# Tencent/PocketFlow

Measured on AMD Instinct MI355X. Metric: images/sec ResNet-50 INT8 quant-aware fine-tune (whole job; per GPU = value / n_gpus), higher is better.
Workload: dtype bf16

## Files before the change

pocketflow_amd/csrc/pf_api.hip:

```cpp
#include "pf_common.h"

extern "C" int pf_version(void) { return 100; }

extern "C" const char* pf_error_string(int err) {
  if (err == 0) return "ok";
  return hipGetErrorString((hipError_t)err);
}

#include <stdlib.h>
#include <stdio.h>
static PfTuning g_tuning;
static bool g_tuning_loaded = false;

static int env_int(const char* name, int dflt) {
  const char* e = getenv(name);
  return (e == nullptr || *e == 0) ? dflt : atoi(e);
}

static void tuning_load() {
  PfTuning t;
  t.conv_bn = env_int("PF_CONV_BN", 0);
  t.conv_igemm = env_int("PF_CONV_IGEMM", 1);
  t.conv_igemm_pro = env_int("PF_CONV_IGEMM_PRO", 1);
  t.conv_stream = env_int("PF_CONV_STREAM", 1);
  t.conv_stream_maxsplit = env_int("PF_CONV_STREAM_MAXSPLIT", 2);
  t.igemm_pro3 = env_int("PF_IGEMM_PRO3", 1);
  t.igemm_tile_bm = t.igemm_tile_bn = 0;
  const char* e = getenv("PF_IGEMM_TILE");
  if (e != nullptr) {
    int bm = 0, bn = 0;
    if (sscanf(e, "%dx%d", &bm, &bn) == 2) { t.igemm_tile_bm = bm; t.igemm_tile_bn = bn; }
  }
  t.pool3s2 = env_int("PF_POOL3S2", 1);
  t.wrw_tr = env_int("PF_WRW_TR", 0);
  t.wrw2 = env_int("PF_WRW2", 1);
  t.wrw2_target = env_int("PF_WRW2_TARGET", 0);
  t.splitk = env_int("PF_IGEMM_SPLITK", 1);
  t.wrw2_tk256 = env_int("PF_WRW2_TK256", 1);
  t.conv3x3_c64 = env_int("PF_CONV3X3_C64", 1);
  g_tuning = t;
  g_tuning_loaded = true;
}

const PfTuning& pf_tuning() {
  if (!g_tuning_loaded) tuning_load();
  return g_tuning;
}

extern "C" int pf_tuning_reload(void) { tuning_load(); return 0; }

#include <map>
#include <mutex>
#include <utility>
int pf_require_lds(const void* fn, size_t lds) {
  static std::mutex mu;
  static std::map<std::pair<int, const void*>, size_t> done;
  int dev = 0;
  hipError_t e = hipGetDevice(&dev);
  if (e != hipSuccess) return (int)e;
  std::lock_guard<std::mutex> lock(mu);
  size_t& have = done[std::make_pair(dev, fn)];
  if (lds > have) {
    e = hipFuncSetAttribute(fn, hipFuncAttributeMaxDynamicSharedMemorySize, (int)lds);
    if (e != hipSuccess) return (int)e;
    have = lds;
  }
  return 0;
}
```

pocketflow_amd/csrc/pf_common.h:

```cpp
#pragma once
#include <hip/hip_runtime.h>
#include <stdint.h>
#include <type_traits>
#include "../../include/pocketflow_hip.h"

#define PF_WAVE 64
#define PF_THREADS 256
#define PF_MAX_GRID 2048

#define PF_LAUNCH_CHECK()                         \
  do {                                            \
    hipError_t e__ = hipGetLastError();           \
    if (e__ != hipSuccess) return (int)e__;       \
  } while (0)

typedef uint16_t bf16_t;

int pf_require_lds(const void* fn, size_t lds);

struct PfTuning {
  int conv_bn;
  int conv_igemm, conv_igemm_pro;
  int conv_stream;
  int conv_stream_maxsplit;
  int igemm_pro3;
  int igemm_tile_bm, igemm_tile_bn;
  int pool3s2;
  int wrw_tr, wrw2, wrw2_target;
  int wrw2_tk256;
  int splitk;
  int conv3x3_c64;
};
const PfTuning& pf_tuning();

__device__ __forceinline__ float bf16_to_f32(bf16_t h) {
  return __uint_as_float(((uint32_t)h) << 16);
}
__device__ __forceinline__ bf16_t f32_to_bf16(float f) {
  uint32_t u = __float_as_uint(f);
  if ((u & 0x7FFFFFFFu) > 0x7F800000u) return (bf16_t)((u >> 16) | 0x0040u);
  u += 0x7FFFu + ((u >> 16) & 1u);
  return (bf16_t)(u >> 16);
}

template <typename T> __device__ __forceinline__ float round_to(float v);
template <> __device__ __forceinline__ float round_to<float>(float v) { return v; }
template <> __device__ __forceinline__ float round_to<bf16_t>(float v) { return bf16_to_f32(f32_to_bf16(v)); }

template <typename T> struct VecTraits;
template <> struct VecTraits<float> { static constexpr int N = 4; };
template <> struct VecTraits<bf16_t> { static constexpr int N = 8; };

template <typename T>
__device__ __forceinline__ void load_vec(const T* __restrict__ p, float* out);
template <>
__device__ __forceinline__ void load_vec<float>(const float* __restrict__ p, float* out) {
  float4 v = *reinterpret_cast<const float4*>(p);
  out[0] = v.x; out[1] = v.y; out[2] = v.z; out[3] = v.w;
}
template <>
__device__ __forceinline__ void load_vec<bf16_t>(const bf16_t* __restrict__ p, float* out) {
  uint4 v = *reinterpret_cast<const uint4*>(p);
  out[0] = __uint_as_float(v.x << 16); out[1] = __uint_as_float(v.x & 0xFFFF0000u);
  out[2] = __uint_as_float(v.y << 16); out[3] = __uint_as_float(v.y & 0xFFFF0000u);
  out[4] = __uint_as_float(v.z << 16); out[5] = __uint_as_float(v.z & 0xFFFF0000u);
  out[6] = __uint_as_float(v.w << 16); out[7] = __uint_as_float(v.w & 0xFFFF0000u);
}
template <typename T>
__device__ __forceinline__ void store_vec(T* __restrict__ p, const float* in);
template <>
__device__ __forceinline__ void store_vec<float>(float* __restrict__ p, const float* in) {
  *reinterpret_cast<float4*>(p) = make_float4(in[0], in[1], in[2], in[3]);
}
template <>
__device__ __forceinline__ void store_vec<bf16_t>(bf16_t* __restrict__ p, const float* in) {
  uint4 v;
  v.x = (uint32_t)f32_to_bf16(in[0]) | ((uint32_t)f32_to_bf16(in[1]) << 16);
  v.y = (uint32_t)f32_to_bf16(in[2]) | ((uint32_t)f32_to_bf16(in[3]) << 16);
  v.z = (uint32_t)f32_to_bf16(in[4]) | ((uint32_t)f32_to_bf16(in[5]) << 16);
  v.w = (uint32_t)f32_to_bf16(in[6]) | ((uint32_t)f32_to_bf16(in[7]) << 16);
  *reinterpret_cast<uint4*>(p) = v;
}
template <typename T> __device__ __forceinline__ void load8(const T* __restrict__ p, float* out);
template <> __device__ __forceinline__ void load8<float>(const float* __restrict__ p, float* out) {
  load_vec<float>(p, out); load_vec<float>(p + 4, out + 4);
}
template <> __device__ __forceinline__ void load8<bf16_t>(const bf16_t* __restrict__ p, float* out) {
  load_vec<bf16_t>(p, out);
}
template <typename T> __device__ __forceinline__ void store8(T* __restrict__ p, const float* in);
template <> __device__ __forceinline__ void store8<float>(float* __restrict__ p, const float* in) {
  store_vec<float>(p, in); store_vec<float>(p + 4, in + 4);
}
template <> __device__ __forceinline__ void store8<bf16_t>(bf16_t* __restrict__ p, const float* in) {
  store_vec<bf16_t>(p, in);
}
__host__ __device__ __forceinline__ bool pf_aligned16(const void* p) {
  return (((uintptr_t)p) & 15) == 0;
}
template <typename T> __device__ __forceinline__ float load_one(const T* p);
template <> __device__ __forceinline__ float load_one<float>(const float* p) { return *p; }
template <> __device__ __forceinline__ float load_one<bf16_t>(const bf16_t* p) { return bf16_to_f32(*p); }
template <typename T> __device__ __forceinline__ void store_one(T* p, float v);
template <> __device__ __forceinline__ void store_one<float>(float* p, float v) { *p = v; }
template <> __device__ __forceinline__ void store_one<bf16_t>(bf16_t* p, float v) { *p = f32_to_bf16(v); }

__device__ __forceinline__ uint32_t enc_f32(float f) {
  uint32_t u = __float_as_uint(f);
  return (u & 0x80000000u) ? ~u : (u | 0x80000000u);
}
__device__ __forceinline__ float dec_f32(uint32_t e) {
  uint32_t u = (e & 0x80000000u) ? (e & 0x7FFFFFFFu) : ~e;
  return __uint_as_float(u);
}
__device__ __forceinline__ void slot_alpha_beta(const uint32_t* slot, float& alpha, float& beta) {
  const uint2 sv = *reinterpret_cast<const uint2*>(slot);
  float mn = dec_f32(sv.x);
  float mx = dec_f32(~sv.y);
  alpha = (mx - mn) + 1e-10f;
  beta = mn;
}

__device__ __forceinline__ float pf_acc_min(float a, float b) { float r; asm("v_min_f32 %0, %1, %2" : "=v"(r) : "v"(a), "v"(b)); return r; }
__device__ __forceinline__ float pf_acc_max(float a, float b) { float r; asm("v_max_f32 %0, %1, %2" : "=v"(r) : "v"(a), "v"(b)); return r; }

template <int ACT> __device__ __forceinline__ float apply_act(float x) {
  if (ACT == PF_ACT_RELU) return fmaxf(x, 0.0f);
  if (ACT == PF_ACT_RELU6) return fminf(fmaxf(x, 0.0f), 6.0f);
  return x;
}
template <int ACT> __device__ __forceinline__ float act_mask(float u) {
  if (ACT == PF_ACT_RELU) return u > 0.0f ? 1.0f : 0.0f;
  if (ACT == PF_ACT_RELU6) return (u > 0.0f && u < 6.0f) ? 1.0f : 0.0f;
  return 1.0f;
}

__device__ __forceinline__ float uq_point(float t, float alpha, float beta, float k) {
  float xn = (t - beta) / alpha;
  float q = rintf(xn * k) / k;
  return alpha * q + beta;
}
__host__ __device__ __forceinline__ float uq_k_of_bits(int bits) {
  return ldexpf(1.0f, bits) - 1.0f;
}

__device__ __forceinline__ float wave_min(float v) {
#pragma unroll
  for (int o = 32; o > 0; o >>= 1) v = fminf(v, __shfl_xor(v, o, 64));
  return v;
}
__device__ __forceinline__ float wave_max(float v) {
#pragma unroll
  for (int o = 32; o > 0; o >>= 1) v = fmaxf(v, __shfl_xor(v, o, 64));
  return v;
}
__device__ __forceinline__ float wave_sum(float v) {
#pragma unroll
  for (int o = 32; o > 0; o >>= 1) v += __shfl_xor(v, o, 64);
  return v;
}
__device__ __forceinline__ void block_minmax(float& mn, float& mx, float* lds ) {
  mn = wave_min(mn);
  mx = wave_max(mx);
  const int w = threadIdx.x >> 6, l = threadIdx.x & 63;
  if (l == 0) { lds[w] = mn; lds[4 + w] = mx; }
  __syncthreads();
  mn = fminf(fminf(lds[0], lds[1]), fminf(lds[2], lds[3]));
  mx = fmaxf(fmaxf(lds[4], lds[5]), fmaxf(lds[6], lds[7]));
  __syncthreads();
}
__device__ __forceinline__ float block_sum(float v, float* lds ) {
  v = wave_sum(v);
  const int w = threadIdx.x >> 6, l = threadIdx.x & 63;
  if (l == 0) lds[w] = v;
  __syncthreads();
  v = (lds[0] + lds[1]) + (lds[2] + lds[3]);
  __syncthreads();
  return v;
}

template <typename F> static inline void pf_with_act(int act, F&& f) {
  if (act == PF_ACT_RELU) f(std::integral_constant<int, PF_ACT_RELU>{});
  else if (act == PF_ACT_RELU6) f(std::integral_constant<int, PF_ACT_RELU6>{});
  else f(std::integral_constant<int, PF_ACT_NONE>{});
}
template <typename F> static inline void pf_with_bool(bool b, F&& f) {
  if (b) f(std::true_type{});
  else f(std::false_type{});
}

static inline int pf_grid_for(int64_t n, int per_block) {
  int64_t g = (n + per_block - 1) / per_block;
  if (g < 1) g = 1;
  if (g > PF_MAX_GRID) g = PF_MAX_GRID;
  return (int)g;
}
```

pocketflow_amd/csrc/pf_igemm.h:

```cpp
#pragma once
#include "pf_conv_common.h"

#define LDS_PTR(p) ((__attribute__((address_space(3))) void*)(p))

#if defined(__HIP_DEVICE_COMPILE__)
typedef __amdgpu_buffer_rsrc_t pf_rsrc_t;
#define PF_MAKE_RSRC(p, bytes) __builtin_amdgcn_make_buffer_rsrc((void*)(p), (short)0, (int)(bytes), 0x00020000)
#define PF_BUFFER_LOAD_LDS16(rs, lds, voff, soff) __builtin_amdgcn_raw_ptr_buffer_load_lds(rs, LDS_PTR(lds), 16, voff, soff, 0, 0)
#else
typedef int pf_rsrc_t;
#define PF_MAKE_RSRC(p, bytes) 0
#define PF_BUFFER_LOAD_LDS16(rs, lds, voff, soff) ((void)(rs), (void)(lds), (void)(voff), (void)(soff))
#endif

struct IgArgs {
  const bf16_t* X;
  const bf16_t* W;
  bf16_t* Y;
  const bf16_t* zero;
  uint32_t x_bytes, w_bytes;
  const bf16_t* R;
  float* partial;
  const bf16_t* bx;
  const float* bss;
  const float* bmi;
  float b_lo, b_hi;
  const float* ss;
  const uint32_t* slot;
  float kq, act_lo, act_hi;
  int M, N, C;
  int th, tw;
  int H, Wd, Ho, Wo, stride, pad_h, pad_w;
  int tiles_m, tiles_n, G;
  int w_r0, w_rs, w_s0, w_ss, w_S, w_taps_full;
  int o_sub, o_y, o_x, o_H, o_W;
  const float* oss;
  int oact;
  int rHo, rWo, rH, rW, rstride;
};

template <int N> __device__ __forceinline__ void wait_vm() { asm volatile("s_waitcnt vmcnt(%0)" ::"n"(N) : "memory"); }

#define IG_PLAIN 0
#define IG_BWD 1
#define IG_PRO 2
```

pocketflow_amd/csrc/pf_igemm.hip:

```cpp
#include "pf_conv_common.h"
#include <stdio.h>
#include <stdlib.h>

#include "pf_igemm.h"

#ifndef PF_IG_ABLATE
#define PF_IG_ABLATE 0
#endif
#define PF_IG_NO_DMA (PF_IG_ABLATE == 2 || PF_IG_ABLATE == 3 || PF_IG_ABLATE == 4)
#define PF_IG_FAKE_FRAGS (PF_IG_ABLATE == 3 || PF_IG_ABLATE == 4)

#ifdef PF_IG_TIMING
#define PF_IG_STAMP(k) do { if (tm_tile == 2) tmk[k] = (uint32_t)__builtin_readcyclecounter(); } while (0)
#else
#define PF_IG_STAMP(k) do { } while (0)
#endif

#ifdef PF_IG_CODES
#define PF_IG_XB 1
__device__ __forceinline__ bf16x8 ig_codes_to_bf16x8(uint2 c) {
  uint32_t r[4];
#pragma unroll
  for (int h = 0; h < 2; ++h) {
    const uint32_t w = h ? c.y : c.x;
    const float f0 = (float)(w & 0xffu), f1 = (float)((w >> 8) & 0xffu), f2 = (float)((w >> 16) & 0xffu), f3 = (float)(w >> 24);
    r[h * 2 + 0] = __builtin_amdgcn_perm(__float_as_uint(f1), __float_as_uint(f0), 0x07060302u);
    r[h * 2 + 1] = __builtin_amdgcn_perm(__float_as_uint(f3), __float_as_uint(f2), 0x07060302u);
  }
  const uint4 u = make_uint4(r[0], r[1], r[2], r[3]);
  return *reinterpret_cast<const bf16x8*>(&u);
}
#else
#define PF_IG_XB 2
#endif

template <int BM, int BN, int WM, int WN, int NS, int MODE, bool SUB = false, bool AFF = false, bool RMAP = false, bool BR = false>
__global__ __launch_bounds__(64 * WM * WN) void k_igemm(const IgArgs a) {
  constexpr bool BWD = (MODE == IG_BWD), PRO = (MODE == IG_PRO);
  static_assert(!BR || BWD, "BR is a variant of IG_BWD");
  static_assert(!PRO || NS == 2 || NS == 3, "the in-LDS prologue pass is written for the 2- and 3-stage rings");
  constexpr bool PRO3 = PRO && NS == 3;
  constexpr int NWC = WM * WN;
  constexpr int T = 64 * NWC;
  constexpr int TS = T;
  constexpr int TE = T;
  constexpr int WR = BM / WM, WC = BN / WN;
  constexpr int JM = WR / 16, NI = WC / 16;
  constexpr int XB = PF_IG_XB;
  constexpr int ACH = 4 * XB, AROW = 64 * XB;
  constexpr int AS = BM * ACH / TS, BS = BN * 8 / TS;
  constexpr int A_BYTES = BM * AROW, B_BYTES = BN * 128, STAGE = A_BYTES + B_BYTES;
  constexpr int CS_LD = BN + 8, CS_LD_B = BN + 8;
  constexpr int VPR = BN / 8, RPP = TE / VPR, NP = BM / RPP;
  static_assert(AS >= 1 && BS >= 1 && NP >= 1, "tile too small for the block");
  constexpr int LPS = AS + BS;
  extern __shared__ __attribute__((aligned(16))) unsigned char smem[];
  bf16_t* Cs = reinterpret_cast<bf16_t*>(smem);
  float* red = reinterpret_cast<float*>(smem);
  constexpr int RING_B = NS * STAGE, CT_B = BM * CS_LD_B * 2;
  float* bpl = reinterpret_cast<float*>(smem + (RING_B > CT_B ? RING_B : CT_B));
  float* ssl = bpl;

  const int tid = threadIdx.x, lane = tid & 63;
  const int wave = __builtin_amdgcn_readfirstlane(tid >> 6);
  const int swave = wave;
  const int cwave = wave % NWC;
  const int wm = cwave / WN, wn = cwave % WN;
  const int l15 = lane & 15, q = lane >> 4;
  const int srow = (swave * 64 + lane) >> 3;
  const int schunk = (lane & 7) ^ ((lane >> 3) & 7);
  const int srowA = (XB == 2) ? srow : ((swave * 64 + lane) >> 2);
  const int schunkA = (XB == 2) ? schunk : ((lane & 3) ^ ((lane >> 4) & 3));

  const int xcd = blockIdx.x & 7, L = blockIdx.x >> 3;
  const int g = xcd + 8 * (L / a.tiles_n), tn = L % a.tiles_n;
  const int n0 = tn * BN;
  const int cch = a.C >> 6;
  const int taps = a.th * a.tw;
  const int nk = taps * cch;
  const int64_t wrow = (int64_t)(SUB ? a.w_taps_full : taps) * a.C;
  const int hw_o = a.Ho * a.Wo;

  if (BWD) {
    for (int i = tid; i < 4 * BN; i += T) {
      const int qq = i / BN, c = n0 + (i - qq * BN);
      float v = 0.f;
      if (c < a.N) v = (qq < 2) ? a.bss[qq * a.N + c] : a.bmi[(qq - 2) * a.N + c];
      bpl[i] = v;
    }
  }

  float st_s[8], st_q[8], st_mn[8], st_mx[8];
#pragma unroll
  for (int j = 0; j < 8; ++j) { st_s[j] = 0.f; st_q[j] = 0.f; st_mn[j] = INFINITY; st_mx[j] = -INFINITY; }
  const int wvec = tid % VPR, wrw = tid / VPR;
  const bf16_t* __restrict__ side = BWD ? a.bx : nullptr;
  Pro pro;
  pro_init(pro, a.act_lo, a.act_hi, a.kq, PRO ? a.slot : nullptr);
  if (PRO3) {
    for (int i = tid; i < 2 * a.C; i += T) ssl[i] = (i < a.C) ? pro_fold_scale(pro, a.ss[i]) : pro_fold_shift(pro, a.ss[i]);
    __syncthreads();
  }

  const pf_rsrc_t rsX = PF_MAKE_RSRC(a.X, a.x_bytes);
  const pf_rsrc_t rsW = PF_MAKE_RSRC(a.W, a.w_bytes);
  constexpr uint32_t OOB = 0x80000000u;
  uint32_t boff[BS];
#pragma unroll
  for (int i = 0; i < BS; ++i) {
    const int n = n0 + i * (TS / 8) + srow;
    boff[i] = (n < a.N) ? (uint32_t)(((int64_t)n * wrow + schunk * 8) * 2) : OOB;
  }

  const bool pointwise = a.th == 1 && a.tw == 1 && a.stride == 1 && a.pad_h == 0 && a.pad_w == 0 && a.Ho == a.H && a.Wo == a.Wd;
  constexpr bool XPRE = !BWD && NS == 3 && 2 * STAGE >= BM * CS_LD_B * 2;
  constexpr int RB0 = XPRE ? 2 : 0;
  uint32_t pbase[AS], pmask[AS];
  int s_r = 0, s_s = 0, s_cc = 0, s_ks = 0, s_tap = 0;
  auto setup_tile = [&](int m0) {
#pragma unroll
    for (int i = 0; i < AS; ++i) {
      const int m = m0 + i * (TS / ACH) + srowA;
      pbase[i] = 0; pmask[i] = 0;
      if (pointwise) {
        if (m < a.M) { pbase[i] = (uint32_t)(m * a.C + schunkA * (16 / XB)) * (uint32_t)XB; pmask[i] = 1u; }
      } else if (m < a.M) {
        const int img = m / hw_o, rem = m - img * hw_o;
        const int ho = rem / a.Wo, wo = rem - ho * a.Wo;
        const int h0 = ho * a.stride - a.pad_h, w0 = wo * a.stride - a.pad_w;
        pbase[i] = (uint32_t)(((img * a.H + h0) * a.Wd + w0) * a.C + schunkA * (16 / XB)) * (uint32_t)XB;
        uint32_t mk = 0;
        for (int r = 0; r < a.th; ++r)
          for (int sx = 0; sx < a.tw; ++sx)
            if ((unsigned)(h0 + r) < (unsigned)a.H && (unsigned)(w0 + sx) < (unsigned)a.Wd) mk |= 1u << (r * a.tw + sx);
        pmask[i] = mk;
      }
    }
    s_r = 0; s_s = 0; s_cc = 0; s_ks = 0; s_tap = 0;
  };
  auto stage = [&](int buf) {
    unsigned char* As = smem + buf * STAGE;
    unsigned char* Bs = As + A_BYTES;
    const uint32_t tapoff = (uint32_t)(((s_r * a.Wd + s_s) * a.C + s_cc * 64) * XB);
#if !PF_IG_NO_DMA
#pragma unroll
    for (int i = 0; i < AS; ++i) {
      const uint32_t voff = ((pmask[i] >> s_tap) & 1u) ? (pbase[i] + tapoff) : OOB;
      PF_BUFFER_LOAD_LDS16(rsX, As + (i * (TS / ACH) + swave * (64 / ACH)) * AROW, voff, 0);
    }
    uint32_t woff = (uint32_t)(s_ks * 128);
    if constexpr (SUB) woff = (uint32_t)((((a.w_r0 + s_r * a.w_rs) * a.w_S + a.w_s0 + s_s * a.w_ss) * a.C + s_cc * 64) * 2);
#pragma unroll
    for (int i = 0; i < BS; ++i)
      PF_BUFFER_LOAD_LDS16(rsW, Bs + (i * (TS / 8) + swave * 8) * 128, boff[i], woff);
#else
    (void)As; (void)Bs; (void)tapoff;
#endif
    ++s_ks;
    if (++s_cc == cch) { s_cc = 0; ++s_tap; if (++s_s == a.tw) { s_s = 0; ++s_r; } }
  };
  bool pre = false;
#ifdef PF_IG_TIMING
  uint32_t tmk[16];
  int tm_tile = -1;
#pragma unroll
  for (int k = 0; k < 16; ++k) tmk[k] = 0;
#endif
  for (int tm = g; tm < a.tiles_m; tm += a.G) {
    const int m0 = tm * BM;
#ifdef PF_IG_TIMING
    ++tm_tile;
#endif
    PF_IG_STAMP(0);
    if (!pre) setup_tile(m0);

    f32x4 acc[NI][JM];
#pragma unroll
    for (int i = 0; i < NI; ++i)
#pragma unroll
      for (int j = 0; j < JM; ++j) acc[i][j] = (f32x4){0.f, 0.f, 0.f, 0.f};
    uint2 rr[NI][JM];
    const bool has_r = BWD ? BR : (a.R != nullptr);
    constexpr bool RPRE = BM * BN <= 128 * 256;
    auto load_residual = [&]() {
#pragma unroll
      for (int j = 0; j < JM; ++j) {
        const int m = m0 + wm * WR + j * 16 + l15;
        int64_t rrow = m;
        bool live = m < a.M;
        if constexpr (RMAP) {
          rrow = live ? rmap_row(m, a.rHo, a.rWo, a.rH, a.rW, a.rstride) : -1;
          live = rrow >= 0;
        }
#pragma unroll
        for (int i = 0; i < NI; ++i) {
          const int n = n0 + wn * WC + i * 16 + q * 4;
          rr[i][j] = make_uint2(0, 0);
          if (live && n < a.N) rr[i][j] = *reinterpret_cast<const uint2*>(a.R + rrow * a.N + n);
        }
      }
    };
    auto add_residual = [&](auto& c) {
#pragma unroll
      for (int j = 0; j < JM; ++j)
#pragma unroll
        for (int i = 0; i < NI; ++i) {
          c[i][j][0] += __uint_as_float(rr[i][j].x << 16); c[i][j][1] += __uint_as_float(rr[i][j].x & 0xFFFF0000u);
          c[i][j][2] += __uint_as_float(rr[i][j].y << 16); c[i][j][3] += __uint_as_float(rr[i][j].y & 0xFFFF0000u);
        }
    };

    int ibuf = RB0;
    float4 ps0 = make_float4(0, 0, 0, 0), ps1 = ps0, ph0 = ps0, ph1 = ps0;
    auto fetch_ss = [&](int cc) {
      const float* p = a.ss + cc * 64 + schunk * 8;
      ps0 = *reinterpret_cast<const float4*>(p); ps1 = *reinterpret_cast<const float4*>(p + 4);
      ph0 = *reinterpret_cast<const float4*>(p + a.C); ph1 = *reinterpret_cast<const float4*>(p + a.C + 4);
    };
    auto transform3 = [&](int buf, int cc, int i0, int i1) {
      const uint32_t pss = lds_addr(ssl + cc * 64 + schunk * 8);
      float4 s0, s1, h0, h1;
      if (i1 - i0 == 1 || i1 - i0 == 2) {
        const uint32_t pd = lds_addr(smem + buf * STAGE + srow * 128 + (lane & 7) * 16) + (uint32_t)(i0 * (TS / 8) * 128);
        uint4 v0, v1 = make_uint4(0, 0, 0, 0);
        if (i1 - i0 == 1) lds_read_b128x4_1(pss, pss + (uint32_t)a.C * 4u, pd, s0, s1, h0, h1, v0);
        else lds_read_b128x4_2(pss, pss + (uint32_t)a.C * 4u, pd, pd + (TS / 8) * 128, s0, s1, h0, h1, v0, v1);
        pro.sc[0] = s0.x; pro.sc[1] = s0.y; pro.sc[2] = s0.z; pro.sc[3] = s0.w;
        pro.sc[4] = s1.x; pro.sc[5] = s1.y; pro.sc[6] = s1.z; pro.sc[7] = s1.w;
        pro.sh[0] = h0.x; pro.sh[1] = h0.y; pro.sh[2] = h0.z; pro.sh[3] = h0.w;
        pro.sh[4] = h1.x; pro.sh[5] = h1.y; pro.sh[6] = h1.z; pro.sh[7] = h1.w;
        lds_write_b128(pd, pro_apply(pro, v0));
        if (i1 - i0 == 2) lds_write_b128(pd + (TS / 8) * 128, pro_apply(pro, v1));
        return;
      }
      lds_read_b128x4(pss, pss + (uint32_t)a.C * 4u, s0, s1, h0, h1);
      pro.sc[0] = s0.x; pro.sc[1] = s0.y; pro.sc[2] = s0.z; pro.sc[3] = s0.w;
      pro.sc[4] = s1.x; pro.sc[5] = s1.y; pro.sc[6] = s1.z; pro.sc[7] = s1.w;
      pro.sh[0] = h0.x; pro.sh[1] = h0.y; pro.sh[2] = h0.z; pro.sh[3] = h0.w;
      pro.sh[4] = h1.x; pro.sh[5] = h1.y; pro.sh[6] = h1.z; pro.sh[7] = h1.w;
      const uint32_t pv = lds_addr(smem + buf * STAGE + srow * 128 + (lane & 7) * 16);
      static_assert(!PRO3 || AS == 1 || AS == 2 || AS == 4 || AS == 8, "vector count per lane");
#pragma unroll
      for (int i = 0; i < AS; i += 2) {
        if (i >= i0 && i < i1) {
          if (i + 1 < i1) {
            uint4 v0, v1;
            lds_read_b128x2(pv + i * (TS / 8) * 128, pv + (i + 1) * (TS / 8) * 128, v0, v1);
            lds_write_b128(pv + i * (TS / 8) * 128, pro_apply(pro, v0));
            lds_write_b128(pv + (i + 1) * (TS / 8) * 128, pro_apply(pro, v1));
          } else {
            lds_write_b128(pv + i * (TS / 8) * 128, pro_apply(pro, lds_read_b128(pv + i * (TS / 8) * 128)));
          }
        } else if (i + 1 >= i0 && i + 1 < i1) {
          lds_write_b128(pv + (i + 1) * (TS / 8) * 128, pro_apply(pro, lds_read_b128(pv + (i + 1) * (TS / 8) * 128)));
        }
      }
    };
    auto transform = [&](int buf) {
      const float rs[8] = {ps0.x, ps0.y, ps0.z, ps0.w, ps1.x, ps1.y, ps1.z, ps1.w};
      const float rh[8] = {ph0.x, ph0.y, ph0.z, ph0.w, ph1.x, ph1.y, ph1.z, ph1.w};
#pragma unroll
      for (int j = 0; j < 8; ++j) { pro.sc[j] = pro_fold_scale(pro, rs[j]); pro.sh[j] = pro_fold_shift(pro, rh[j]); }
      unsigned char* As = smem + buf * STAGE;
#pragma unroll
      for (int i = 0; i < AS; ++i) {
        uint4* p = reinterpret_cast<uint4*>(As + (i * (TS / 8) + srow) * 128 + (lane & 7) * 16);
        *p = pro_apply(pro, *p);
      }
    };
    {
#pragma unroll
    for (int d = 0; d < NS - 1; ++d)
      if (d < nk) {
        if (d > 0 || !pre) {
          if (PRO && !PRO3) fetch_ss(s_cc);
          stage(ibuf);
        }
        ibuf = (ibuf + 1 == NS) ? 0 : ibuf + 1;
      }
    PF_IG_STAMP(1);
    if (nk >= NS - 1) wait_vm<(NS - 2) * LPS>(); else wait_vm<0>();
    PF_IG_STAMP(2);
    if (PRO3) { transform3(RB0, 0, 0, AS); asm volatile("s_waitcnt lgkmcnt(0)" ::: "memory"); }
    else if (PRO) { transform(RB0); asm volatile("s_waitcnt lgkmcnt(0)" ::: "memory"); }
    __builtin_amdgcn_s_barrier();
    PF_IG_STAMP(3);
    int cbuf = RB0;
    for (int ks = 0; ks < nk; ++ks) {
      const bool more = ks + NS - 1 < nk;
      const int tbuf = ibuf;
      if (more) {
        if (PRO && !PRO3) fetch_ss(s_cc);
        stage(ibuf);
        ibuf = (ibuf + 1 == NS) ? 0 : ibuf + 1;
      }
      const unsigned char* As = smem + cbuf * STAGE;
      const unsigned char* Bs = As + A_BYTES;
      cbuf = (cbuf + 1 == NS) ? 0 : cbuf + 1;
      const bool tnext = PRO3 && (ks + 1 < nk);
      if (PRO3) {
        if (more) wait_vm<LPS>(); else if (ks + 1 < nk) wait_vm<0>();
      }
      if (RPRE && has_r && ks == ((PRO3 && nk >= 2) ? nk - 2 : nk - 1)) load_residual();
#pragma unroll
      for (int kk = 0; kk < 2; ++kk) {
        const int coff = (((kk * 4 + q) ^ (l15 & 7)) << 4);
        bf16x8 wf[NI], xf[JM];
#if PF_IG_ABLATE != 1
#if PF_IG_FAKE_FRAGS
#pragma unroll
        for (int i = 0; i < NI; ++i) { uint4 u = make_uint4(lane, i, kk, 0x3f803f80u); asm volatile("" : "+v"(u.x)); wf[i] = *reinterpret_cast<const bf16x8*>(&u); }
#pragma unroll
        for (int j = 0; j < JM; ++j) { uint4 u = make_uint4(lane, j, kk, 0x3f803f80u); asm volatile("" : "+v"(u.x)); xf[j] = *reinterpret_cast<const bf16x8*>(&u); }
        (void)coff;
#else
#pragma unroll
        for (int i = 0; i < NI; ++i)
          wf[i] = *reinterpret_cast<const bf16x8*>(Bs + (wn * WC + i * 16 + l15) * 128 + coff);
#ifdef PF_IG_CODES
        const int coffA = ((((kk * 2 + (q >> 1)) ^ ((l15 >> 2) & 3)) << 4) + (q & 1) * 8);
#pragma unroll
        for (int j = 0; j < JM; ++j)
          xf[j] = ig_codes_to_bf16x8(*reinterpret_cast<const uint2*>(As + (wm * WR + j * 16 + l15) * AROW + coffA));
#else
#pragma unroll
        for (int j = 0; j < JM; ++j)
          xf[j] = *reinterpret_cast<const bf16x8*>(As + (wm * WR + j * 16 + l15) * 128 + coff);
#endif
#endif
#pragma unroll
        for (int i = 0; i < NI; ++i)
#pragma unroll
          for (int j = 0; j < JM; ++j)
            acc[i][j] = __builtin_amdgcn_mfma_f32_16x16x32_bf16(wf[i], xf[j], acc[i][j], 0, 0, 0);
        if constexpr (NI == 4 && JM == 4 && PRO3) {
          __builtin_amdgcn_sched_group_barrier(0x100, NI + JM, 0);
          __builtin_amdgcn_sched_group_barrier(0x008, NI * JM, 0);
        }
        if constexpr ((NI == 4 || NI == 2) && JM == 4 && !PRO3) {
          if (kk == 1) {
            __builtin_amdgcn_sched_group_barrier(0x100, NI + JM, 0);
#pragma unroll
            for (int i = 0; i < NI + JM; ++i) {
              __builtin_amdgcn_sched_group_barrier(0x008, (NI * JM) / (NI + JM), 0);
              __builtin_amdgcn_sched_group_barrier(0x100, 1, 0);
            }
            __builtin_amdgcn_sched_group_barrier(0x008, NI * JM - (NI + JM) * ((NI * JM) / (NI + JM)) + NI * JM, 0);
          }
        }
#else
        (void)coff; (void)wf; (void)xf;
#endif
        if (tnext) transform3(cbuf, ks + 1, kk * (AS / 2), (kk == 1) ? AS : (AS / 2));
      }
      if (!PRO3) {
        if (more) wait_vm<(NS - 2) * LPS>(); else wait_vm<0>();
      }
      if (PRO && !PRO3 && more) transform(tbuf);
      asm volatile("s_waitcnt lgkmcnt(0)" ::: "memory");
      __builtin_amdgcn_s_barrier();
      __builtin_amdgcn_sched_barrier(0);
#ifdef PF_IG_TIMING
      if (ks < 4) PF_IG_STAMP(4 + ks);
      if (ks == nk - 1) PF_IG_STAMP(8);
#endif
    }
    }

#if PF_IG_ABLATE >= 4
    {
      if (a.M < 0) {
#pragma unroll
        for (int i = 0; i < NI; ++i)
#pragma unroll
          for (int j = 0; j < JM; ++j) reinterpret_cast<uint32_t*>(a.Y)[(i * JM + j) * 64 + lane] = pack_bf16x2(acc[i][j][0] + acc[i][j][1], acc[i][j][2] + acc[i][j][3]);
      }
      continue;
    }
#endif
    {
    if (has_r) {
      if constexpr (RPRE) add_residual(acc);
      else {
#pragma unroll
        for (int j = 0; j < JM; ++j) {
          const int m = m0 + wm * WR + j * 16 + l15;
          int64_t rrow = m;
          bool live = m < a.M;
          if constexpr (RMAP) {
            rrow = live ? rmap_row(m, a.rHo, a.rWo, a.rH, a.rW, a.rstride) : -1;
            live = rrow >= 0;
          }
#pragma unroll
          for (int i = 0; i < NI; ++i) {
            const int n = n0 + wn * WC + i * 16 + q * 4;
            if (live && n < a.N) {
              const uint2 r = *reinterpret_cast<const uint2*>(a.R + rrow * a.N + n);
              acc[i][j][0] += __uint_as_float(r.x << 16); acc[i][j][1] += __uint_as_float(r.x & 0xFFFF0000u);
              acc[i][j][2] += __uint_as_float(r.y << 16); acc[i][j][3] += __uint_as_float(r.y & 0xFFFF0000u);
            }
          }
          __builtin_amdgcn_sched_barrier(0);
        }
      }
    }
    PF_IG_STAMP(9);
    pre = false;
    if constexpr (XPRE) {
      __builtin_amdgcn_sched_barrier(0);
      if (tm + a.G < a.tiles_m) {
        setup_tile((tm + a.G) * BM);
        stage(RB0);
        pre = true;
      }
      __builtin_amdgcn_sched_barrier(0);
    }
#ifdef PF_IG_CODES
#pragma unroll
    for (int i = 0; i < NI; ++i)
#pragma unroll
      for (int j = 0; j < JM; ++j)
#pragma unroll
        for (int e = 0; e < 4; ++e) acc[i][j][e] *= a.kq;
#endif
#pragma unroll
    for (int i = 0; i < NI; ++i)
#pragma unroll
      for (int j = 0; j < JM; ++j) {
        const uint2 v = make_uint2(pack_bf16x2(acc[i][j][0], acc[i][j][1]), pack_bf16x2(acc[i][j][2], acc[i][j][3]));
        if constexpr (XPRE) lds_write_b64(lds_addr(Cs + (wm * WR + j * 16 + l15) * CS_LD + wn * WC + i * 16 + q * 4), v);
        else *reinterpret_cast<uint2*>(Cs + (wm * WR + j * 16 + l15) * CS_LD + wn * WC + i * 16 + q * 4) = v;
      }
    }
    constexpr int PG = (NP > 8) ? 8 : NP;
    uint4 rres[PG];
    auto load_side = [&](int p0) {
#pragma unroll
      for (int p = 0; p < PG; ++p) {
        const int m = m0 + wrw + (p0 + p) * RPP, n = n0 + wvec * 8;
        rres[p] = make_uint4(0, 0, 0, 0);
        if (m < a.M && n < a.N) {
          int64_t srow = m;
          if constexpr (SUB) {
            const int oimg = m / hw_o, orem = m - oimg * hw_o;
            const int oi = orem / a.Wo, oj = orem - oi * a.Wo;
            srow = ((int64_t)oimg * a.o_H + oi * a.o_sub + a.o_y) * a.o_W + oj * a.o_sub + a.o_x;
          }
          rres[p] = *reinterpret_cast<const uint4*>(side + srow * a.N + n);
        }
      }
    };
    constexpr bool etid = true;
    float bpr[32];
    if (BWD && !BR) {
#pragma unroll
      for (int qq = 0; qq < 4; ++qq)
#pragma unroll
        for (int j = 0; j < 8; ++j) bpr[qq * 8 + j] = bpl[qq * BN + wvec * 8 + j];
    }
    if (side != nullptr && etid) load_side(0);
    PF_IG_STAMP(10);
    if constexpr (XPRE) { asm volatile("s_waitcnt lgkmcnt(0)" ::: "memory"); __builtin_amdgcn_s_barrier(); __builtin_amdgcn_sched_barrier(0); }
    else __syncthreads();
    PF_IG_STAMP(11);
#pragma unroll
    for (int p0 = 0; p0 < NP; p0 += PG) {
      u32x4_t cv[8];
      if constexpr (XPRE && PG == 8) {
#pragma unroll
        for (int pp = 0; pp < PG; ++pp) lds_read_b128_nowait(lds_addr(Cs + (wrw + (p0 + pp) * RPP) * CS_LD + wvec * 8), cv[pp]);
        lds_wait_batch8(cv);
      } else {
#pragma unroll
        for (int pp = 0; pp < PG; ++pp) cv[pp] = *reinterpret_cast<const u32x4_t*>(Cs + (wrw + (p0 + pp) * RPP) * CS_LD + wvec * 8);
      }
#pragma unroll
      for (int pp = 0; pp < PG; ++pp) {
        const int p = p0 + pp;
        const int rl = wrw + p * RPP;
        const int m = m0 + rl, n = n0 + wvec * 8;
        if (m < a.M && n < a.N && etid) {
          uint4 c;
          c = make_uint4(cv[pp][0], cv[pp][1], cv[pp][2], cv[pp][3]);
          if (BWD) {
            float f[8], xv[8];
            unpack8(c, f);
            unpack8(rres[pp], xv);
            const float* bp = BR ? (bpl + wvec * 8) : bpr;
            constexpr int BPS = BR ? BN : 8;
#pragma unroll
            for (int j = 0; j < 8; ++j) {
              const float u = fmaf(bp[j], xv[j], bp[BPS + j]);
              const float dy = (u > a.b_lo && u < a.b_hi) ? f[j] : 0.f;
              st_s[j] += dy;
              st_q[j] = fmaf(dy, (xv[j] - bp[2 * BPS + j]) * bp[3 * BPS + j], st_q[j]);
            }
          } else if (a.R != nullptr || a.partial != nullptr) {
            float f[8];
            unpack8(c, f);
            if (a.partial != nullptr) {
#pragma unroll
              for (int j = 0; j < 8; ++j) {
                st_s[j] += f[j];
                st_q[j] = fmaf(f[j], f[j], st_q[j]);
                st_mn[j] = pf_acc_min(st_mn[j], f[j]);
                st_mx[j] = pf_acc_max(st_mx[j], f[j]);
              }
            }
          }
          if constexpr (AFF) c = out_affine8(c, a.oss, a.N, n, a.oact);
          int64_t orow = m;
          if constexpr (SUB) {
            const int oimg = m / hw_o, orem = m - oimg * hw_o;
            const int oi = orem / a.Wo, oj = orem - oi * a.Wo;
            orow = ((int64_t)oimg * a.o_H + oi * a.o_sub + a.o_y) * a.o_W + oj * a.o_sub + a.o_x;
          }
          *reinterpret_cast<uint4*>(a.Y + orow * a.N + n) = c;
        }
      }
      if (side != nullptr && p0 + PG < NP && etid) load_side(p0 + PG);
    }
    PF_IG_STAMP(12);
    if constexpr (XPRE) { asm volatile("s_waitcnt lgkmcnt(0)" ::: "memory"); __builtin_amdgcn_s_barrier(); __builtin_amdgcn_sched_barrier(0); }
    else __syncthreads();
    PF_IG_STAMP(13);
#ifdef PF_IG_TIMING
    if (tm_tile == 2 && blockIdx.x == gridDim.x / 2 && tid == 0) {
      uint32_t* out = reinterpret_cast<uint32_t*>(const_cast<bf16_t*>(a.zero));
#pragma unroll
      for (int k = 0; k < 14; ++k) out[k] = tmk[k];
      out[14] = (uint32_t)__builtin_readcyclecounter();
    }
#endif
  }

  if (a.partial != nullptr) {
    constexpr int nstat_max = 4;
    const int nstat = BWD ? 2 : 4;
    __syncthreads();
    for (int stat = 0; stat < nstat; ++stat) {
      const float* v = (stat == 0) ? st_s : (stat == 1 ? st_q : (stat == 2 ? st_mn : st_mx));
#pragma unroll
      for (int j = 0; j < 8; ++j) red[wrw * BN + wvec * 8 + j] = v[j];
      __syncthreads();
      for (int c = tid; c < BN; c += T) {
        float r = red[c];
        for (int rr = 1; rr < RPP; ++rr) {
          const float w = red[rr * BN + c];
          r = (stat < 2) ? (r + w) : (stat == 2 ? fminf(r, w) : fmaxf(r, w));
        }
        if (n0 + c < a.N) a.partial[((int64_t)g * nstat + stat) * a.N + n0 + c] = r;
      }
      __syncthreads();
    }
    (void)nstat_max;
  }
}

static IgCfg ig_pick(int M, int N, bool pro) {
  if (pro) {
    if (pf_tuning().igemm_pro3 != 0) {
      if (N % 256 == 0) return IgCfg{128, 256, 256, true};
      if (N % 128 == 0) return IgCfg{256, 128, 256, true};
    }
    return IgCfg{128, (N % 128 == 0) ? 128 : 64, 512, false};
  }
  {
    const int bm = pf_tuning().igemm_tile_bm, bn = pf_tuning().igemm_tile_bn;
    if ((bm == 128 || bm == 256) && (bn == 64 || bn == 128) && (N % bn == 0 || bn == 64))
      return IgCfg{bm, bn, (bm == 256) ? 256 : 512, false};
  }
  const int bn = (N % 128 == 0) ? 128 : 64;
  return IgCfg{128, bn, 512, false};
}

static IgArgs ig_args_plain(int th, int tw) {
  IgArgs a;
  a.X = nullptr; a.W = nullptr; a.Y = nullptr; a.zero = nullptr; a.x_bytes = 0; a.w_bytes = 0;
  a.R = nullptr; a.partial = nullptr; a.bx = nullptr; a.bss = nullptr; a.bmi = nullptr; a.b_lo = -INFINITY; a.b_hi = INFINITY;
  a.ss = nullptr; a.slot = nullptr; a.kq = 255.f; a.act_lo = -INFINITY; a.act_hi = INFINITY;
  a.M = 0; a.N = 0; a.C = 0; a.th = th; a.tw = tw;
  a.H = 1; a.Wd = 1; a.Ho = 1; a.Wo = 1; a.stride = 1; a.pad_h = 0; a.pad_w = 0;
  a.tiles_m = 0; a.tiles_n = 0; a.G = 0;
  a.w_r0 = 0; a.w_rs = 1; a.w_s0 = 0; a.w_ss = 1; a.w_S = tw; a.w_taps_full = th * tw;
  a.o_sub = 0; a.o_y = 0; a.o_x = 0; a.o_H = 0; a.o_W = 0;
  a.oss = nullptr; a.oact = PF_ACT_NONE;
  a.rHo = 0; a.rWo = 0; a.rH = 0; a.rW = 0; a.rstride = 1;
  return a;
}

template <int BM, int BN, int WM, int WN, int NS, int MODE, bool SUB = false, bool AFF = false, bool RMAP = false, bool BR = false>
static int ig_launch_t(IgArgs& a, int slots, hipStream_t st) {
  constexpr bool BWD = (MODE == IG_BWD), PRO3 = (MODE == IG_PRO && NS == 3);
  constexpr int THREADS = 64 * WM * WN;
  a.tiles_m = (a.M + BM - 1) / BM;
  a.tiles_n = (a.N + BN - 1) / BN;
  const int planned_G = a.G;
  const int grid = pf_conv_grid(slots, a.tiles_m, a.tiles_n, &a.G);
  if (planned_G > 0 && a.G != planned_G) return (int)hipErrorInvalidValue;
  constexpr size_t ring = NS * (size_t)(BM + BN) * 128, ctile = (size_t)BM * (BN + 8) * 2;
  constexpr size_t base = (ring > ctile ? ring : ctile);
  const size_t lds = base + (BWD ? 4 * BN * 4 : 0) + (PRO3 ? 2 * (size_t)a.C * 4 : 0);
  if (PRO3 && a.C > CV_MAXK) return (int)hipErrorInvalidValue;
  const size_t lds_max = base + (BWD ? 4 * BN * 4 : 0) + (PRO3 ? 2 * (size_t)CV_MAXK * 4 : 0);
  if (int e = pf_require_lds(reinterpret_cast<const void*>(&k_igemm<BM, BN, WM, WN, NS, MODE, SUB, AFF, RMAP, BR>), lds_max)) return e;
  k_igemm<BM, BN, WM, WN, NS, MODE, SUB, AFF, RMAP, BR><<<grid, THREADS, lds, st>>>(a);
  PF_LAUNCH_CHECK();
  return 0;
}

bool pf_conv3x3_c64_geom(int H, int Wd, int C, int N, int th, int tw, int stride, int pad_h, int pad_w, int Ho, int Wo);
bool pf_conv3x3_c64_takes(const IgArgs& a);
int pf_conv3x3_c64_stats_groups(int M);
int pf_conv3x3_c64_launch(const IgArgs& a, hipStream_t st);

static bool ig_carries_affine(const IgCfg& c, bool pro, int taps) { return pro ? (c.pro3 && taps == 1) : c.bm == 128; }

static int ig_launch(IgArgs& a, const IgCfg& c, hipStream_t st) {
  const bool bwd = a.bx != nullptr, pro = a.ss != nullptr;
  if (pf_conv3x3_c64_takes(a)) return pf_conv3x3_c64_launch(a, st);
  if (a.oss != nullptr) {
    if (bwd) return (int)hipErrorInvalidValue;
    if (!ig_carries_affine(c, pro, a.th * a.tw)) {
      const float* oss = a.oss;
      a.oss = nullptr;
      const int r = ig_launch(a, c, st);
      if (r != 0) return r;
      return pf_bn_act_quant_apply(a.Y, a.Y, PF_BF16, a.M, a.N, oss, a.oact, nullptr, 8, 0, st);
    }
    if (pro) return (c.bn == 256) ? ig_launch_t<128, 256, 2, 4, 3, IG_PRO, false, true>(a, c.slots, st)
                                  : ig_launch_t<256, 128, 4, 2, 3, IG_PRO, false, true>(a, c.slots, st);
    return (c.bn == 128) ? ig_launch_t<128, 128, 2, 2, 2, IG_PLAIN, false, true>(a, c.slots, st)
                         : ig_launch_t<128, 64, 2, 2, 2, IG_PLAIN, false, true>(a, c.slots, st);
  }
  if (pro) {
    if (a.th * a.tw != 1 || bwd) return (int)hipErrorInvalidValue;
    if (c.pro3) return (c.bn == 256) ? ig_launch_t<128, 256, 2, 4, 3, IG_PRO>(a, c.slots, st)
                                     : ig_launch_t<256, 128, 4, 2, 3, IG_PRO>(a, c.slots, st);
    return (c.bn == 128) ? ig_launch_t<128, 128, 2, 2, 2, IG_PRO>(a, c.slots, st) : ig_launch_t<128, 64, 2, 2, 2, IG_PRO>(a, c.slots, st);
  }
#define PF_IG(BMV, BNV, WMV, WNV, NSV) (bwd ? ig_launch_t<BMV, BNV, WMV, WNV, NSV, IG_BWD>(a, c.slots, st) : ig_launch_t<BMV, BNV, WMV, WNV, NSV, IG_PLAIN>(a, c.slots, st))
  if (c.bm == 256 && c.bn == 128) return PF_IG(256, 128, 4, 2, 3);
  if (c.bm == 128 && c.bn == 128) return PF_IG(128, 128, 2, 2, 2);
  if (c.bm == 256 && c.bn == 64) return PF_IG(256, 64, 4, 1, 2);
  return PF_IG(128, 64, 2, 2, 2);
#undef PF_IG
}

extern "C" int pf_conv2d_stats_groups_geom(int imgs, int H, int Wd, int C, int N, int th, int tw, int stride, int pad_h,
                                           int pad_w, int Ho, int Wo) {
  if (pf_conv3x3_c64_geom(H, Wd, C, N, th, tw, stride, pad_h, pad_w, Ho, Wo) && (imgs * Ho * Wo) % (Ho * Wo) == 0)
    return pf_conv3x3_c64_stats_groups(imgs * Ho * Wo);
  const int M = imgs * Ho * Wo;
  const IgCfg c = ig_pick(M, N, false);
  int G;
  pf_conv_grid(c.slots, (M + c.bm - 1) / c.bm, (N + c.bn - 1) / c.bn, &G);
  return G;
}

static int conv2d_fwd_launch(const void* X, const void* W, void* Y, const void* zero, const void* R, float* partial,
                             const void* bn_x, const float* bn_scale_shift, const float* bn_mean_invstd, int bn_act,
                             int imgs, int H, int Wd, int C, int N, int th, int tw, int stride, int pad_h, int pad_w,
                             int Ho, int Wo, void* stream, const float* out_scale_shift, int out_act) {
  if (out_scale_shift != nullptr && (R != nullptr || partial != nullptr || bn_x != nullptr)) return (int)hipErrorInvalidValue;
  if (imgs <= 0 || H <= 0 || Wd <= 0 || Ho <= 0 || Wo <= 0 || C <= 0 || N <= 0 || (C % 64) || (N % 8) || th < 1 || tw < 1 ||
      stride < 1)
    return (int)hipErrorInvalidValue;
  if (!pf_aligned16(X) || !pf_aligned16(W) || !pf_aligned16(Y) || !pf_aligned16(zero) || zero == nullptr ||
      (R && !pf_aligned16(R)) || (bn_x && !pf_aligned16(bn_x)))
    return (int)hipErrorInvalidValue;
  if (bn_x != nullptr && (R != nullptr || partial == nullptr || bn_scale_shift == nullptr || bn_mean_invstd == nullptr))
    return (int)hipErrorInvalidValue;
  if ((int64_t)imgs * H * Wd * C >= ((int64_t)1 << 30) || (int64_t)N * th * tw * C >= ((int64_t)1 << 30) || th * tw > 32)
    return (int)hipErrorInvalidValue;
  IgArgs a = ig_args_plain(th, tw);
  a.X = (const bf16_t*)X; a.W = (const bf16_t*)W; a.Y = (bf16_t*)Y; a.zero = (const bf16_t*)zero;
  a.R = (const bf16_t*)R; a.partial = partial; a.bx = (const bf16_t*)bn_x; a.bss = bn_scale_shift; a.bmi = bn_mean_invstd;
  pf_act_window(bn_act, &a.b_lo, &a.b_hi);
  a.M = imgs * Ho * Wo; a.N = N; a.C = C;
  a.H = H; a.Wd = Wd; a.Ho = Ho; a.Wo = Wo; a.stride = stride; a.pad_h = pad_h; a.pad_w = pad_w;
  a.x_bytes = (uint32_t)((int64_t)imgs * H * Wd * C * 2);
  a.w_bytes = (uint32_t)((int64_t)N * th * tw * C * 2);
  a.oss = out_scale_shift; a.oact = out_act;
  return ig_launch(a, ig_pick(a.M, N, false), (hipStream_t)stream);
}

extern "C" int pf_conv2d_fwd(const void* X, const void* W, void* Y, const void* zero, const void* R, float* partial,
                             const void* bn_x, const float* bn_scale_shift, const float* bn_mean_invstd, int bn_act,
                             int imgs, int H, int Wd, int C, int N, int th, int tw, int stride, int pad_h, int pad_w,
                             int Ho, int Wo, void* stream) {
  return conv2d_fwd_launch(X, W, Y, zero, R, partial, bn_x, bn_scale_shift, bn_mean_invstd, bn_act, imgs, H, Wd, C, N, th, tw,
                           stride, pad_h, pad_w, Ho, Wo, stream, nullptr, PF_ACT_NONE);
}

#ifdef PF_IG_CODES
extern "C" int pf_probe_conv2d_fwd_codes(const void* Xc, float alpha, const void* W, void* Y, const void* zero, int imgs, int H,
                                         int Wd, int C, int N, int th, int tw, int stride, int pad_h, int pad_w, int Ho, int Wo,
                                         void* stream) {
  if ((C % 64) || (N % 64) || !pf_aligned16(Xc) || !pf_aligned16(W) || !pf_aligned16(Y)) return (int)hipErrorInvalidValue;
  IgArgs a = ig_args_plain(th, tw);
  a.X = (const bf16_t*)Xc; a.W = (const bf16_t*)W; a.Y = (bf16_t*)Y; a.zero = (const bf16_t*)zero;
  a.kq = alpha;
  a.M = imgs * Ho * Wo; a.N = N; a.C = C;
  a.H = H; a.Wd = Wd; a.Ho = Ho; a.Wo = Wo; a.stride = stride; a.pad_h = pad_h; a.pad_w = pad_w;
  a.x_bytes = (uint32_t)((int64_t)imgs * H * Wd * C);
  a.w_bytes = (uint32_t)((int64_t)N * th * tw * C * 2);
  const IgCfg c = ig_pick(a.M, a.N, false);
  if (c.bm == 256 && c.bn == 128) return ig_launch_t<256, 128, 4, 2, 3, IG_PLAIN>(a, c.slots, (hipStream_t)stream);
  if (c.bm == 128 && c.bn == 128) return ig_launch_t<128, 128, 2, 2, 2, IG_PLAIN>(a, c.slots, (hipStream_t)stream);
  if (c.bm == 256 && c.bn == 64) return ig_launch_t<256, 64, 4, 1, 2, IG_PLAIN>(a, c.slots, (hipStream_t)stream);
  return ig_launch_t<128, 64, 2, 2, 2, IG_PLAIN>(a, c.slots, (hipStream_t)stream);
}
#endif

extern "C" int pf_conv2d_fwd_affine(const void* X, const void* W, void* Y, const void* zero, const float* out_scale_shift,
                                    int out_act, int imgs, int H, int Wd, int C, int N, int th, int tw, int stride, int pad_h,
                                    int pad_w, int Ho, int Wo, void* stream) {
  if (out_scale_shift == nullptr) return (int)hipErrorInvalidValue;
  return conv2d_fwd_launch(X, W, Y, zero, nullptr, nullptr, nullptr, nullptr, nullptr, PF_ACT_NONE, imgs, H, Wd, C, N, th, tw,
                           stride, pad_h, pad_w, Ho, Wo, stream, out_scale_shift, out_act);
}

static int strided_class_groups(int imgs, int H, int Wd, int C, int stride) {
  const int bn = (C % 128 == 0) ? 128 : 64;
  int G;
  pf_conv_grid(512, (imgs * (H / stride) * (Wd / stride) + 127) / 128, (C + bn - 1) / bn, &G);
  return G;
}

extern "C" int pf_conv2d_bwd_data_strided_stats_groups(int imgs, int H, int Wd, int C, int stride) {
  if (imgs <= 0 || H <= 0 || Wd <= 0 || C <= 0 || stride < 2 || (H % stride) || (Wd % stride)) return 0;
  return stride * stride * strided_class_groups(imgs, H, Wd, C, stride);
}

static int strided_launch(const void* dY, const void* Wt, void* dX, const void* zero, int imgs, int H, int Wd, int C, int N, int R,
                          int S, int stride, int pad_h, int pad_w, int Ho, int Wo, void* stream, float* partial, const void* bn_x,
                          const float* bss, const float* bmi, int bn_act) {
  if (imgs <= 0 || H <= 0 || Wd <= 0 || Ho <= 0 || Wo <= 0 || C <= 0 || N <= 0 || (N % 64) || (C % 8) || stride < 2 || R < stride ||
      S < stride || (H % stride) || (Wd % stride) || pad_h < 0 || pad_w < 0 || R * S > 32)
    return (int)hipErrorInvalidValue;
  if (!pf_aligned16(dY) || !pf_aligned16(Wt) || !pf_aligned16(dX) || zero == nullptr) return (int)hipErrorInvalidValue;
  if ((int64_t)imgs * Ho * Wo * N >= ((int64_t)1 << 30) || (int64_t)C * R * S * N >= ((int64_t)1 << 30)) return (int)hipErrorInvalidValue;
  const int Hc = H / stride, Wc = Wd / stride;
  for (int ay = 0; ay < stride; ++ay) {
    for (int ax = 0; ax < stride; ++ax) {
      const int r1 = (ay + pad_h) % stride, s1 = (ax + pad_w) % stride;
      const int th = (R - r1 + stride - 1) / stride, tw = (S - s1 + stride - 1) / stride;
      const int dmin_h = (ay + pad_h - r1) / stride - (th - 1), dmin_w = (ax + pad_w - s1) / stride - (tw - 1);
      IgArgs a = ig_args_plain(th, tw);
      a.X = (const bf16_t*)dY; a.W = (const bf16_t*)Wt; a.Y = (bf16_t*)dX; a.zero = (const bf16_t*)zero;
      if (bn_x != nullptr) {
        a.partial = partial + (int64_t)(ay * stride + ax) * strided_class_groups(imgs, H, Wd, C, stride) * 2 * C;
        a.bx = (const bf16_t*)bn_x; a.bss = bss; a.bmi = bmi;
        pf_act_window(bn_act, &a.b_lo, &a.b_hi);
      }
      a.M = imgs * Hc * Wc; a.N = C; a.C = N;
      a.H = Ho; a.Wd = Wo; a.Ho = Hc; a.Wo = Wc; a.stride = 1; a.pad_h = -dmin_h; a.pad_w = -dmin_w;
      a.x_bytes = (uint32_t)((int64_t)imgs * Ho * Wo * N * 2);
      a.w_bytes = (uint32_t)((int64_t)C * R * S * N * 2);
      a.w_r0 = (R - 1 - r1) - (th - 1) * stride; a.w_rs = stride;
      a.w_s0 = (S - 1 - s1) - (tw - 1) * stride; a.w_ss = stride;
      a.w_S = S; a.w_taps_full = R * S;
      a.o_sub = stride; a.o_y = ay; a.o_x = ax; a.o_H = H; a.o_W = Wd;
      int rc;
      if (bn_x != nullptr)
        rc = (C % 128 == 0) ? ig_launch_t<128, 128, 2, 2, 2, IG_BWD, true>(a, 512, (hipStream_t)stream)
                            : ig_launch_t<128, 64, 2, 2, 2, IG_BWD, true>(a, 512, (hipStream_t)stream);
      else
        rc = (C % 128 == 0) ? ig_launch_t<128, 128, 2, 2, 2, IG_PLAIN, true>(a, 512, (hipStream_t)stream)
                            : ig_launch_t<128, 64, 2, 2, 2, IG_PLAIN, true>(a, 512, (hipStream_t)stream);
      if (rc != 0) return rc;
    }
  }
  return 0;
}

extern "C" int pf_conv2d_bwd_data_strided(const void* dY, const void* Wt, void* dX, const void* zero, int imgs, int H, int Wd,
                                          int C, int N, int R, int S, int stride, int pad_h, int pad_w, int Ho, int Wo, void* stream) {
  return strided_launch(dY, Wt, dX, zero, imgs, H, Wd, C, N, R, S, stride, pad_h, pad_w, Ho, Wo, stream, nullptr, nullptr, nullptr,
                        nullptr, PF_ACT_NONE);
}

extern "C" int pf_conv2d_bwd_data_strided_bnstats(const void* dY, const void* Wt, void* dX, const void* zero, const void* bn_x,
                                                  const float* bn_scale_shift, const float* bn_mean_invstd, int bn_act,
                                                  float* partial, int imgs, int H, int Wd, int C, int N, int R, int S, int stride,
                                                  int pad_h, int pad_w, int Ho, int Wo, void* stream) {
  if (bn_x == nullptr || partial == nullptr || bn_scale_shift == nullptr || bn_mean_invstd == nullptr || !pf_aligned16(bn_x))
    return (int)hipErrorInvalidValue;
  return strided_launch(dY, Wt, dX, zero, imgs, H, Wd, C, N, R, S, stride, pad_h, pad_w, Ho, Wo, stream, partial, bn_x,
                        bn_scale_shift, bn_mean_invstd, bn_act);
}

bool pf_igemm_conv1x1_plan(const Conv1x1Req& q, Conv1x1Plan* p) {
  const int64_t lim = (int64_t)1 << 30;
  if ((q.K % 64) || q.rows_in * q.K >= lim || (int64_t)q.N * q.K >= lim) return false;
  IgCfg c = ig_pick(q.M, q.N, q.pro);
  if (q.join) {
    if ((q.N % 64) || c.bm != 128 || c.slots != 512 || c.bn != ((q.N % 128 == 0) ? 128 : 64)) return false;
    if (q.ymap || q.map || !q.res || q.pro || q.aff) return false;
  } else if (q.ymap) {
    if ((q.N % 64) || q.rows_out * q.N >= lim) return false;
    c = IgCfg{128, (q.N % 128 == 0) ? 128 : 64, 512, false};
  }
  p->kernel = CONV_IGEMM;
  p->ig = c;
  p->grid = pf_conv_grid(c.slots, (q.M + c.bm - 1) / c.bm, (q.N + c.bn - 1) / c.bn, &p->G);
  p->rows_in = q.rows_in;
  p->affine_after = q.aff && !ig_carries_affine(c, q.pro, 1);
  return true;
}

int pf_igemm_conv1x1(const ConvArgs& c, const Conv1x1Plan& p, hipStream_t st) {
  const bool rowmap = c.stride > 1 && !c.ymap;
  IgArgs a = ig_args_plain(1, 1);
  a.X = c.X; a.W = c.W; a.Y = c.Y; a.zero = c.X;
#ifdef PF_IG_TIMING
  a.zero = (const bf16_t*)(uintptr_t)strtoull(getenv("PF_IG_TIMING_PTR"), nullptr, 0);
#endif
  a.R = c.R; a.partial = c.partial; a.bx = c.bx; a.bss = c.bss; a.bmi = c.bmi; a.b_lo = c.b_lo; a.b_hi = c.b_hi;
  a.ss = c.ss; a.slot = c.slot; a.kq = c.kq; a.act_lo = c.act_lo; a.act_hi = c.act_hi;
  a.M = c.M; a.N = c.N; a.C = c.K; a.G = p.G;
  if (c.ymap) { a.H = c.Ho; a.Wd = c.Wo; a.Ho = c.Ho; a.Wo = c.Wo; }
  else if (rowmap) { a.H = c.H; a.Wd = c.Wd; a.Ho = c.Ho; a.Wo = c.Wo; a.stride = c.stride; }
  a.x_bytes = (uint32_t)(p.rows_in * c.K * 2);
  a.w_bytes = (uint32_t)((int64_t)c.N * c.K * 2);
  a.oss = c.oss; a.oact = c.oact;
  a.rHo = c.rHo; a.rWo = c.rWo; a.rH = c.rH; a.rW = c.rW; a.rstride = c.rstride;
  const bool rmap = a.rstride > 1, br = a.bx != nullptr && a.R != nullptr, wide = (p.ig.bn == 128);
  if (rmap || br) {
    if (!br) return wide ? ig_launch_t<128, 128, 2, 2, 2, IG_PLAIN, false, false, true, false>(a, 512, st)
                         : ig_launch_t<128, 64, 2, 2, 2, IG_PLAIN, false, false, true, false>(a, 512, st);
    if (rmap) return wide ? ig_launch_t<128, 128, 2, 2, 2, IG_BWD, false, false, true, true>(a, 512, st)
                          : ig_launch_t<128, 64, 2, 2, 2, IG_BWD, false, false, true, true>(a, 512, st);
    return wide ? ig_launch_t<128, 128, 2, 2, 2, IG_BWD, false, false, false, true>(a, 512, st)
                : ig_launch_t<128, 64, 2, 2, 2, IG_BWD, false, false, false, true>(a, 512, st);
  }
  if (c.ymap) {
    a.o_sub = c.stride; a.o_y = 0; a.o_x = 0; a.o_H = c.H; a.o_W = c.Wd;
    return wide ? ig_launch_t<128, 128, 2, 2, 2, IG_PLAIN, true>(a, 512, st) : ig_launch_t<128, 64, 2, 2, 2, IG_PLAIN, true>(a, 512, st);
  }
  return ig_launch(a, p.ig, st);
}
```

Before: 11620.

## Fuse strided backward-data sub-convolution classes into a single kernel launch

Adds an IgSubArgs struct carrying up to 16 per-phase sub-class descriptors (tap offsets, padding, output offsets, partial pointers). The igemm kernel now loops over these classes internally, so a strided transposed convolution needs one launch instead of one per phase. This targets the per-launch overhead and the tail effects of many small grids. In exchange the kernel grows larger, and per-block work becomes uneven when classes have different tap counts.

```diff
diff --git a/pocketflow_amd/csrc/pf_api.hip b/pocketflow_amd/csrc/pf_api.hip
--- a/pocketflow_amd/csrc/pf_api.hip
+++ b/pocketflow_amd/csrc/pf_api.hip
@@ -38,6 +38,7 @@
   t.splitk = env_int("PF_IGEMM_SPLITK", 1);
   t.wrw2_tk256 = env_int("PF_WRW2_TK256", 1);
   t.conv3x3_c64 = env_int("PF_CONV3X3_C64", 1);
+  t.strided_one_launch = env_int("PF_STRIDED_ONE_LAUNCH", 1);
   g_tuning = t;
   g_tuning_loaded = true;
 }
diff --git a/pocketflow_amd/csrc/pf_common.h b/pocketflow_amd/csrc/pf_common.h
--- a/pocketflow_amd/csrc/pf_common.h
+++ b/pocketflow_amd/csrc/pf_common.h
@@ -30,6 +30,7 @@
   int wrw2_tk256;
   int splitk;
   int conv3x3_c64;
+  int strided_one_launch;
 };
 const PfTuning& pf_tuning();
 
diff --git a/pocketflow_amd/csrc/pf_igemm.h b/pocketflow_amd/csrc/pf_igemm.h
--- a/pocketflow_amd/csrc/pf_igemm.h
+++ b/pocketflow_amd/csrc/pf_igemm.h
@@ -12,6 +12,16 @@
 #define PF_MAKE_RSRC(p, bytes) 0
 #define PF_BUFFER_LOAD_LDS16(rs, lds, voff, soff) ((void)(rs), (void)(lds), (void)(voff), (void)(soff))
 #endif
+
+#define IG_MAX_CLS 16
+struct IgSubCls {
+  int th, tw, pad_h, pad_w;
+  int w_r0, w_s0;
+  int o_y, o_x;
+  int rot;
+  int pad_;
+  float* partial;
+};
 
 struct IgArgs {
   const bf16_t* X;
@@ -39,6 +49,12 @@
   int rHo, rWo, rH, rW, rstride;
 };
 
+struct IgSubArgs : IgArgs {
+  int n_cls;
+  IgSubCls cls[IG_MAX_CLS];
+};
+template <bool SUB, class A> __device__ __forceinline__ const A& ig_sub_args(const A& a) { return a; }
+
 template <int N> __device__ __forceinline__ void wait_vm() { asm volatile("s_waitcnt vmcnt(%0)" ::"n"(N) : "memory"); }
 
 #define IG_PLAIN 0
diff --git a/pocketflow_amd/csrc/pf_igemm.hip b/pocketflow_amd/csrc/pf_igemm.hip
--- a/pocketflow_amd/csrc/pf_igemm.hip
+++ b/pocketflow_amd/csrc/pf_igemm.hip
@@ -36,525 +36,14 @@
 
 template <int BM, int BN, int WM, int WN, int NS, int MODE, bool SUB = false, bool AFF = false, bool RMAP = false, bool BR = false>
 __global__ __launch_bounds__(64 * WM * WN) void k_igemm(const IgArgs a) {
-  constexpr bool BWD = (MODE == IG_BWD), PRO = (MODE == IG_PRO);
-  static_assert(!BR || BWD, "BR is a variant of IG_BWD");
-  static_assert(!PRO || NS == 2 || NS == 3, "the in-LDS prologue pass is written for the 2- and 3-stage rings");
-  constexpr bool PRO3 = PRO && NS == 3;
-  constexpr int NWC = WM * WN;
-  constexpr int T = 64 * NWC;
-  constexpr int TS = T;
-  constexpr int TE = T;
-  constexpr int WR = BM / WM, WC = BN / WN;
-  constexpr int JM = WR / 16, NI = WC / 16;
-  constexpr int XB = PF_IG_XB;
-  constexpr int ACH = 4 * XB, AROW = 64 * XB;
-  constexpr int AS = BM * ACH / TS, BS = BN * 8 / TS;
-  constexpr int A_BYTES = BM * AROW, B_BYTES = BN * 128, STAGE = A_BYTES + B_BYTES;
-  constexpr int CS_LD = BN + 8, CS_LD_B = BN + 8;
-  constexpr int VPR = BN / 8, RPP = TE / VPR, NP = BM / RPP;
-  static_assert(AS >= 1 && BS >= 1 && NP >= 1, "tile too small for the block");
-  constexpr int LPS = AS + BS;
-  extern __shared__ __attribute__((aligned(16))) unsigned char smem[];
-  bf16_t* Cs = reinterpret_cast<bf16_t*>(smem);
-  float* red = reinterpret_cast<float*>(smem);
-  constexpr int RING_B = NS * STAGE, CT_B = BM * CS_LD_B * 2;
-  float* bpl = reinterpret_cast<float*>(smem + (RING_B > CT_B ? RING_B : CT_B));
-  float* ssl = bpl;
-
-  const int tid = threadIdx.x, lane = tid & 63;
-  const int wave = __builtin_amdgcn_readfirstlane(tid >> 6);
-  const int swave = wave;
-  const int cwave = wave % NWC;
-  const int wm = cwave / WN, wn = cwave % WN;
-  const int l15 = lane & 15, q = lane >> 4;
-  const int srow = (swave * 64 + lane) >> 3;
-  const int schunk = (lane & 7) ^ ((lane >> 3) & 7);
-  const int srowA = (XB == 2) ? srow : ((swave * 64 + lane) >> 2);
-  const int schunkA = (XB == 2) ? schunk : ((lane & 3) ^ ((lane >> 4) & 3));
-
-  const int xcd = blockIdx.x & 7, L = blockIdx.x >> 3;
-  const int g = xcd + 8 * (L / a.tiles_n), tn = L % a.tiles_n;
-  const int n0 = tn * BN;
-  const int cch = a.C >> 6;
-  const int taps = a.th * a.tw;
-  const int nk = taps * cch;
-  const int64_t wrow = (int64_t)(SUB ? a.w_taps_full : taps) * a.C;
-  const int hw_o = a.Ho * a.Wo;
-
-  if (BWD) {
-    for (int i = tid; i < 4 * BN; i += T) {
-      const int qq = i / BN, c = n0 + (i - qq * BN);
-      float v = 0.f;
-      if (c < a.N) v = (qq < 2) ? a.bss[qq * a.N + c] : a.bmi[(qq - 2) * a.N + c];
-      bpl[i] = v;
-    }
-  }
-
-  float st_s[8], st_q[8], st_mn[8], st_mx[8];
-#pragma unroll
-  for (int j = 0; j < 8; ++j) { st_s[j] = 0.f; st_q[j] = 0.f; st_mn[j] = INFINITY; st_mx[j] = -INFINITY; }
-  const int wvec = tid % VPR, wrw = tid / VPR;
-  const bf16_t* __restrict__ side = BWD ? a.bx : nullptr;
-  Pro pro;
-  pro_init(pro, a.act_lo, a.act_hi, a.kq, PRO ? a.slot : nullptr);
-  if (PRO3) {
-    for (int i = tid; i < 2 * a.C; i += T) ssl[i] = (i < a.C) ? pro_fold_scale(pro, a.ss[i]) : pro_fold_shift(pro, a.ss[i]);
-    __syncthreads();
-  }
-
-  const pf_rsrc_t rsX = PF_MAKE_RSRC(a.X, a.x_bytes);
-  const pf_rsrc_t rsW = PF_MAKE_RSRC(a.W, a.w_bytes);
-  constexpr uint32_t OOB = 0x80000000u;
-  uint32_t boff[BS];
-#pragma unroll
-  for (int i = 0; i < BS; ++i) {
-    const int n = n0 + i * (TS / 8) + srow;
-    boff[i] = (n < a.N) ? (uint32_t)(((int64_t)n * wrow + schunk * 8) * 2) : OOB;
-  }
-
-  const bool pointwise = a.th == 1 && a.tw == 1 && a.stride == 1 && a.pad_h == 0 && a.pad_w == 0 && a.Ho == a.H && a.Wo == a.Wd;
-  constexpr bool XPRE = !BWD && NS == 3 && 2 * STAGE >= BM * CS_LD_B * 2;
-  constexpr int RB0 = XPRE ? 2 : 0;
-  uint32_t pbase[AS], pmask[AS];
-  int s_r = 0, s_s = 0, s_cc = 0, s_ks = 0, s_tap = 0;
-  auto setup_tile = [&](int m0) {
-#pragma unroll
-    for (int i = 0; i < AS; ++i) {
-      const int m = m0 + i * (TS / ACH) + srowA;
-      pbase[i] = 0; pmask[i] = 0;
-      if (pointwise) {
-        if (m < a.M) { pbase[i] = (uint32_t)(m * a.C + schunkA * (16 / XB)) * (uint32_t)XB; pmask[i] = 1u; }
-      } else if (m < a.M) {
-        const int img = m / hw_o, rem = m - img * hw_o;
-        const int ho = rem / a.Wo, wo = rem - ho * a.Wo;
-        const int h0 = ho * a.stride - a.pad_h, w0 = wo * a.stride - a.pad_w;
-        pbase[i] = (uint32_t)(((img * a.H + h0) * a.Wd + w0) * a.C + schunkA * (16 / XB)) * (uint32_t)XB;
-        uint32_t mk = 0;
-        for (int r = 0; r < a.th; ++r)
-          for (int sx = 0; sx < a.tw; ++sx)
-            if ((unsigned)(h0 + r) < (unsigned)a.H && (unsigned)(w0 + sx) < (unsigned)a.Wd) mk |= 1u << (r * a.tw + sx);
-        pmask[i] = mk;
-      }
-    }
-    s_r = 0; s_s = 0; s_cc = 0; s_ks = 0; s_tap = 0;
-  };
-  auto stage = [&](int buf) {
-    unsigned char* As = smem + buf * STAGE;
-    unsigned char* Bs = As + A_BYTES;
-    const uint32_t tapoff = (uint32_t)(((s_r * a.Wd + s_s) * a.C + s_cc * 64) * XB);
-#if !PF_IG_NO_DMA
-#pragma unroll
-    for (int i = 0; i < AS; ++i) {
-      const uint32_t voff = ((pmask[i] >> s_tap) & 1u) ? (pbase[i] + tapoff) : OOB;
-      PF_BUFFER_LOAD_LDS16(rsX, As + (i * (TS / ACH) + swave * (64 / ACH)) * AROW, voff, 0);
-    }
-    uint32_t woff = (uint32_t)(s_ks * 128);
-    if constexpr (SUB) woff = (uint32_t)((((a.w_r0 + s_r * a.w_rs) * a.w_S + a.w_s0 + s_s * a.w_ss) * a.C + s_cc * 64) * 2);
-#pragma unroll
-    for (int i = 0; i < BS; ++i)
-      PF_BUFFER_LOAD_LDS16(rsW, Bs + (i * (TS / 8) + swave * 8) * 128, boff[i], woff);
-#else
-    (void)As; (void)Bs; (void)tapoff;
-#endif
-    ++s_ks;
-    if (++s_cc == cch) { s_cc = 0; ++s_tap; if (++s_s == a.tw) { s_s = 0; ++s_r; } }
-  };
-  bool pre = false;
-#ifdef PF_IG_TIMING
-  uint32_t tmk[16];
-  int tm_tile = -1;
-#pragma unroll
-  for (int k = 0; k < 16; ++k) tmk[k] = 0;
-#endif
-  for (int tm = g; tm < a.tiles_m; tm += a.G) {
-    const int m0 = tm * BM;
-#ifdef PF_IG_TIMING
-    ++tm_tile;
-#endif
-    PF_IG_STAMP(0);
-    if (!pre) setup_tile(m0);
-
-    f32x4 acc[NI][JM];
-#pragma unroll
-    for (int i = 0; i < NI; ++i)
-#pragma unroll
-      for (int j = 0; j < JM; ++j) acc[i][j] = (f32x4){0.f, 0.f, 0.f, 0.f};
-    uint2 rr[NI][JM];
-    const bool has_r = BWD ? BR : (a.R != nullptr);
-    constexpr bool RPRE = BM * BN <= 128 * 256;
-    auto load_residual = [&]() {
-#pragma unroll
-      for (int j = 0; j < JM; ++j) {
-        const int m = m0 + wm * WR + j * 16 + l15;
-        int64_t rrow = m;
-        bool live = m < a.M;
-        if constexpr (RMAP) {
-          rrow = live ? rmap_row(m, a.rHo, a.rWo, a.rH, a.rW, a.rstride) : -1;
-          live = rrow >= 0;
-        }
-#pragma unroll
-        for (int i = 0; i < NI; ++i) {
-          const int n = n0 + wn * WC + i * 16 + q * 4;
-          rr[i][j] = make_uint2(0, 0);
-          if (live && n < a.N) rr[i][j] = *reinterpret_cast<const uint2*>(a.R + rrow * a.N + n);
-        }
-      }
-    };
-    auto add_residual = [&](auto& c) {
-#pragma unroll
-      for (int j = 0; j < JM; ++j)
-#pragma unroll
-        for (int i = 0; i < NI; ++i) {
-          c[i][j][0] += __uint_as_float(rr[i][j].x << 16); c[i][j][1] += __uint_as_float(rr[i][j].x & 0xFFFF0000u);
-          c[i][j][2] += __uint_as_float(rr[i][j].y << 16); c[i][j][3] += __uint_as_float(rr[i][j].y & 0xFFFF0000u);
-        }
-    };
-
-    int ibuf = RB0;
-    float4 ps0 = make_float4(0, 0, 0, 0), ps1 = ps0, ph0 = ps0, ph1 = ps0;
-    auto fetch_ss = [&](int cc) {
-      const float* p = a.ss + cc * 64 + schunk * 8;
-      ps0 = *reinterpret_cast<const float4*>(p); ps1 = *reinterpret_cast<const float4*>(p + 4);
-      ph0 = *reinterpret_cast<const float4*>(p + a.C); ph1 = *reinterpret_cast<const float4*>(p + a.C + 4);
-    };
-    auto transform3 = [&](int buf, int cc, int i0, int i1) {
-      const uint32_t pss = lds_addr(ssl + cc * 64 + schunk * 8);
-      float4 s0, s1, h0, h1;
-      if (i1 - i0 == 1 || i1 - i0 == 2) {
-        const uint32_t pd = lds_addr(smem + buf * STAGE + srow * 128 + (lane & 7) * 16) + (uint32_t)(i0 * (TS / 8) * 128);
-        uint4 v0, v1 = make_uint4(0, 0, 0, 0);
-        if (i1 - i0 == 1) lds_read_b128x4_1(pss, pss + (uint32_t)a.C * 4u, pd, s0, s1, h0, h1, v0);
-        else lds_read_b128x4_2(pss, pss + (uint32_t)a.C * 4u, pd, pd + (TS / 8) * 128, s0, s1, h0, h1, v0, v1);
-        pro.sc[0] = s0.x; pro.sc[1] = s0.y; pro.sc[2] = s0.z; pro.sc[3] = s0.w;
-        pro.sc[4] = s1.x; pro.sc[5] = s1.y; pro.sc[6] = s1.z; pro.sc[7] = s1.w;
-        pro.sh[0] = h0.x; pro.sh[1] = h0.y; pro.sh[2] = h0.z; pro.sh[3] = h0.w;
-        pro.sh[4] = h1.x; pro.sh[5] = h1.y; pro.sh[6] = h1.z; pro.sh[7] = h1.w;
-        lds_write_b128(pd, pro_apply(pro, v0));
-        if (i1 - i0 == 2) lds_write_b128(pd + (TS / 8) * 128, pro_apply(pro, v1));
-        return;
-      }
-      lds_read_b128x4(pss, pss + (uint32_t)a.C * 4u, s0, s1, h0, h1);
-      pro.sc[0] = s0.x; pro.sc[1] = s0.y; pro.sc[2] = s0.z; pro.sc[3] = s0.w;
-      pro.sc[4] = s1.x; pro.sc[5] = s1.y; pro.sc[6] = s1.z; pro.sc[7] = s1.w;
-      pro.sh[0] = h0.x; pro.sh[1] = h0.y; pro.sh[2] = h0.z; pro.sh[3] = h0.w;
-      pro.sh[4] = h1.x; pro.sh[5] = h1.y; pro.sh[6] = h1.z; pro.sh[7] = h1.w;
-      const uint32_t pv = lds_addr(smem + buf * STAGE + srow * 128 + (lane & 7) * 16);
-      static_assert(!PRO3 || AS == 1 || AS == 2 || AS == 4 || AS == 8, "vector count per lane");
-#pragma unroll
-      for (int i = 0; i < AS; i += 2) {
-        if (i >= i0 && i < i1) {
-          if (i + 1 < i1) {
-            uint4 v0, v1;
-            lds_read_b128x2(pv + i * (TS / 8) * 128, pv + (i + 1) * (TS / 8) * 128, v0, v1);
-            lds_write_b128(pv + i * (TS / 8) * 128, pro_apply(pro, v0));
-            lds_write_b128(pv + (i + 1) * (TS / 8) * 128, pro_apply(pro, v1));
-          } else {
-            lds_write_b128(pv + i * (TS / 8) * 128, pro_apply(pro, lds_read_b128(pv + i * (TS / 8) * 128)));
-          }
-        } else if (i + 1 >= i0 && i + 1 < i1) {
-          lds_write_b128(pv + (i + 1) * (TS / 8) * 128, pro_apply(pro, lds_read_b128(pv + (i + 1) * (TS / 8) * 128)));
-        }
-      }
-    };
-    auto transform = [&](int buf) {
-      const float rs[8] = {ps0.x, ps0.y, ps0.z, ps0.w, ps1.x, ps1.y, ps1.z, ps1.w};
-      const float rh[8] = {ph0.x, ph0.y, ph0.z, ph0.w, ph1.x, ph1.y, ph1.z, ph1.w};
-#pragma unroll
-      for (int j = 0; j < 8; ++j) { pro.sc[j] = pro_fold_scale(pro, rs[j]); pro.sh[j] = pro_fold_shift(pro, rh[j]); }
-      unsigned char* As = smem + buf * STAGE;
-#pragma unroll
-      for (int i = 0; i < AS; ++i) {
-        uint4* p = reinterpret_cast<uint4*>(As + (i * (TS / 8) + srow) * 128 + (lane & 7) * 16);
-        *p = pro_apply(pro, *p);
-      }
-    };
-    {
-#pragma unroll
-    for (int d = 0; d < NS - 1; ++d)
-      if (d < nk) {
-        if (d > 0 || !pre) {
-          if (PRO && !PRO3) fetch_ss(s_cc);
-          stage(ibuf);
-        }
-        ibuf = (ibuf + 1 == NS) ? 0 : ibuf + 1;
-      }
-    PF_IG_STAMP(1);
-    if (nk >= NS - 1) wait_vm<(NS - 2) * LPS>(); else wait_vm<0>();
-    PF_IG_STAMP(2);
-    if (PRO3) { transform3(RB0, 0, 0, AS); asm volatile("s_waitcnt lgkmcnt(0)" ::: "memory"); }
-    else if (PRO) { transform(RB0); asm volatile("s_waitcnt lgkmcnt(0)" ::: "memory"); }
-    __builtin_amdgcn_s_barrier();
-    PF_IG_STAMP(3);
-    int cbuf = RB0;
-    for (int ks = 0; ks < nk; ++ks) {
-      const bool more = ks + NS - 1 < nk;
-      const int tbuf = ibuf;
-      if (more) {
-        if (PRO && !PRO3) fetch_ss(s_cc);
-        stage(ibuf);
-        ibuf = (ibuf + 1 == NS) ? 0 : ibuf + 1;
-      }
-      const unsigned char* As = smem + cbuf * STAGE;
-      const unsigned char* Bs = As + A_BYTES;
-      cbuf = (cbuf + 1 == NS) ? 0 : cbuf + 1;
-      const bool tnext = PRO3 && (ks + 1 < nk);
-      if (PRO3) {
-        if (more) wait_vm<LPS>(); else if (ks + 1 < nk) wait_vm<0>();
-      }
-      if (RPRE && has_r && ks == ((PRO3 && nk >= 2) ? nk - 2 : nk - 1)) load_residual();
-#pragma unroll
-      for (int kk = 0; kk < 2; ++kk) {
-        const int coff = (((kk * 4 + q) ^ (l15 & 7)) << 4);
-        bf16x8 wf[NI], xf[JM];
-#if PF_IG_ABLATE != 1
-#if PF_IG_FAKE_FRAGS
-#pragma unroll
-        for (int i = 0; i < NI; ++i) { uint4 u = make_uint4(lane, i, kk, 0x3f803f80u); asm volatile("" : "+v"(u.x)); wf[i] = *reinterpret_cast<const bf16x8*>(&u); }
-#pragma unroll
-        for (int j = 0; j < JM; ++j) { uint4 u = make_uint4(lane, j, kk, 0x3f803f80u); asm volatile("" : "+v"(u.x)); xf[j] = *reinterpret_cast<const bf16x8*>(&u); }
-        (void)coff;
-#else
-#pragma unroll
-        for (int i = 0; i < NI; ++i)
-          wf[i] = *reinterpret_cast<const bf16x8*>(Bs + (wn * WC + i * 16 + l15) * 128 + coff);
-#ifdef PF_IG_CODES
-        const int coffA = ((((kk * 2 + (q >> 1)) ^ ((l15 >> 2) & 3)) << 4) + (q & 1) * 8);
-#pragma unroll
-        for (int j = 0; j < JM; ++j)
-          xf[j] = ig_codes_to_bf16x8(*reinterpret_cast<const uint2*>(As + (wm * WR + j * 16 + l15) * AROW + coffA));
-#else
-#pragma unroll
-        for (int j = 0; j < JM; ++j)
-          xf[j] = *reinterpret_cast<const bf16x8*>(As + (wm * WR + j * 16 + l15) * 128 + coff);
-#endif
-#endif
-#pragma unroll
-        for (int i = 0; i < NI; ++i)
-#pragma unroll
-          for (int j = 0; j < JM; ++j)
-            acc[i][j] = __builtin_amdgcn_mfma_f32_16x16x32_bf16(wf[i], xf[j], acc[i][j], 0, 0, 0);
-        if constexpr (NI == 4 && JM == 4 && PRO3) {
-          __builtin_amdgcn_sched_group_barrier(0x100, NI + JM, 0);
-          __builtin_amdgcn_sched_group_barrier(0x008, NI * JM, 0);
-        }
-        if constexpr ((NI == 4 || NI == 2) && JM == 4 && !PRO3) {
-          if (kk == 1) {
-            __builtin_amdgcn_sched_group_barrier(0x100, NI + JM, 0);
-#pragma unroll
-            for (int i = 0; i < NI + JM; ++i) {
-              __builtin_amdgcn_sched_group_barrier(0x008, (NI * JM) / (NI + JM), 0);
-              __builtin_amdgcn_sched_group_barrier(0x100, 1, 0);
-            }
-            __builtin_amdgcn_sched_group_barrier(0x008, NI * JM - (NI + JM) * ((NI * JM) / (NI + JM)) + NI * JM, 0);
-          }
-        }
-#else
-        (void)coff; (void)wf; (void)xf;
-#endif
-        if (tnext) transform3(cbuf, ks + 1, kk * (AS / 2), (kk == 1) ? AS : (AS / 2));
-      }
-      if (!PRO3) {
-        if (more) wait_vm<(NS - 2) * LPS>(); else wait_vm<0>();
-      }
-      if (PRO && !PRO3 && more) transform(tbuf);
-      asm volatile("s_waitcnt lgkmcnt(0)" ::: "memory");
-      __builtin_amdgcn_s_barrier();
-      __builtin_amdgcn_sched_barrier(0);
-#ifdef PF_IG_TIMING
-      if (ks < 4) PF_IG_STAMP(4 + ks);
-      if (ks == nk - 1) PF_IG_STAMP(8);
-#endif
-    }
-    }
-
-#if PF_IG_ABLATE >= 4
-    {
-      if (a.M < 0) {
-#pragma unroll
-        for (int i = 0; i < NI; ++i)
-#pragma unroll
-          for (int j = 0; j < JM; ++j) reinterpret_cast<uint32_t*>(a.Y)[(i * JM + j) * 64 + lane] = pack_bf16x2(acc[i][j][0] + acc[i][j][1], acc[i][j][2] + acc[i][j][3]);
-      }
-      continue;
-    }
-#endif
-    {
-    if (has_r) {
-      if constexpr (RPRE) add_residual(acc);
-      else {
-#pragma unroll
-        for (int j = 0; j < JM; ++j) {
-          const int m = m0 + wm * WR + j * 16 + l15;
-          int64_t rrow = m;
-          bool live = m < a.M;
-          if constexpr (RMAP) {
-            rrow = live ? rmap_row(m, a.rHo, a.rWo, a.rH, a.rW, a.rstride) : -1;
-            live = rrow >= 0;
-          }
-#pragma unroll
-          for (int i = 0; i < NI; ++i) {
-            const int n = n0 + wn * WC + i * 16 + q * 4;
-            if (live && n < a.N) {
-              const uint2 r = *reinterpret_cast<const uint2*>(a.R + rrow * a.N + n);
-              acc[i][j][0] += __uint_as_float(r.x << 16); acc[i][j][1] += __uint_as_float(r.x & 0xFFFF0000u);
-              acc[i][j][2] += __uint_as_float(r.y << 16); acc[i][j][3] += __uint_as_float(r.y & 0xFFFF0000u);
-            }
-          }
-          __builtin_amdgcn_sched_barrier(0);
-        }
-      }
-    }
-    PF_IG_STAMP(9);
-    pre = false;
-    if constexpr (XPRE) {
-      __builtin_amdgcn_sched_barrier(0);
-      if (tm + a.G < a.tiles_m) {
-        setup_tile((tm + a.G) * BM);
-        stage(RB0);
-        pre = true;
-      }
-      __builtin_amdgcn_sched_barrier(0);
-    }
-#ifdef PF_IG_CODES
-#pragma unroll
-    for (int i = 0; i < NI; ++i)
-#pragma unroll
-      for (int j = 0; j < JM; ++j)
-#pragma unroll
-        for (int e = 0; e < 4; ++e) acc[i][j][e] *= a.kq;
-#endif
-#pragma unroll
-    for (int i = 0; i < NI; ++i)
-#pragma unroll
-      for (int j = 0; j < JM; ++j) {
-        const uint2 v = make_uint2(pack_bf16x2(acc[i][j][0], acc[i][j][1]), pack_bf16x2(acc[i][j][2], acc[i][j][3]));
-        if constexpr (XPRE) lds_write_b64(lds_addr(Cs + (wm * WR + j * 16 + l15) * CS_LD + wn * WC + i * 16 + q * 4), v);
-        else *reinterpret_cast<uint2*>(Cs + (wm * WR + j * 16 + l15) * CS_LD + wn * WC + i * 16 + q * 4) = v;
-      }
-    }
-    constexpr int PG = (NP > 8) ? 8 : NP;
-    uint4 rres[PG];
-    auto load_side = [&](int p0) {
-#pragma unroll
-      for (int p = 0; p < PG; ++p) {
-        const int m = m0 + wrw + (p0 + p) * RPP, n = n0 + wvec * 8;
-        rres[p] = make_uint4(0, 0, 0, 0);
-        if (m < a.M && n < a.N) {
-          int64_t srow = m;
-          if constexpr (SUB) {
-            const int oimg = m / hw_o, orem = m - oimg * hw_o;
-            const int oi = orem / a.Wo, oj = orem - oi * a.Wo;
-            srow = ((int64_t)oimg * a.o_H + oi * a.o_sub + a.o_y) * a.o_W + oj * a.o_sub + a.o_x;
-          }
-          rres[p] = *reinterpret_cast<const uint4*>(side + srow * a.N + n);
-        }
-      }
-    };
-    constexpr bool etid = true;
-    float bpr[32];
-    if (BWD && !BR) {
-#pragma unroll
-      for (int qq = 0; qq < 4; ++qq)
-#pragma unroll
-        for (int j = 0; j < 8; ++j) bpr[qq * 8 + j] = bpl[qq * BN + wvec * 8 + j];
-    }
-    if (side != nullptr && etid) load_side(0);
-    PF_IG_STAMP(10);
-    if constexpr (XPRE) { asm volatile("s_waitcnt lgkmcnt(0)" ::: "memory"); __builtin_amdgcn_s_barrier(); __builtin_amdgcn_sched_barrier(0); }
-    else __syncthreads();
-    PF_IG_STAMP(11);
-#pragma unroll
-    for (int p0 = 0; p0 < NP; p0 += PG) {
-      u32x4_t cv[8];
-      if constexpr (XPRE && PG == 8) {
-#pragma unroll
-        for (int pp = 0; pp < PG; ++pp) lds_read_b128_nowait(lds_addr(Cs + (wrw + (p0 + pp) * RPP) * CS_LD + wvec * 8), cv[pp]);
-        lds_wait_batch8(cv);
-      } else {
-#pragma unroll
-        for (int pp = 0; pp < PG; ++pp) cv[pp] = *reinterpret_cast<const u32x4_t*>(Cs + (wrw + (p0 + pp) * RPP) * CS_LD + wvec * 8);
-      }
-#pragma unroll
-      for (int pp = 0; pp < PG; ++pp) {
-        const int p = p0 + pp;
-        const int rl = wrw + p * RPP;
-        const int m = m0 + rl, n = n0 + wvec * 8;
-        if (m < a.M && n < a.N && etid) {
-          uint4 c;
-          c = make_uint4(cv[pp][0], cv[pp][1], cv[pp][2], cv[pp][3]);
-          if (BWD) {
-            float f[8], xv[8];
-            unpack8(c, f);
-            unpack8(rres[pp], xv);
-            const float* bp = BR ? (bpl + wvec * 8) : bpr;
-            constexpr int BPS = BR ? BN : 8;
-#pragma unroll
-            for (int j = 0; j < 8; ++j) {
-              const float u = fmaf(bp[j], xv[j], bp[BPS + j]);
-              const float dy = (u > a.b_lo && u < a.b_hi) ? f[j] : 0.f;
-              st_s[j] += dy;
-              st_q[j] = fmaf(dy, (xv[j] - bp[2 * BPS + j]) * bp[3 * BPS + j], st_q[j]);
-            }
-          } else if (a.R != nullptr || a.partial != nullptr) {
-            float f[8];
-            unpack8(c, f);
-            if (a.partial != nullptr) {
-#pragma unroll
-              for (int j = 0; j < 8; ++j) {
-                st_s[j] += f[j];
-                st_q[j] = fmaf(f[j], f[j], st_q[j]);
-                st_mn[j] = pf_acc_min(st_mn[j], f[j]);
-                st_mx[j] = pf_acc_max(st_mx[j], f[j]);
-              }
-            }
-          }
-          if constexpr (AFF) c = out_affine8(c, a.oss, a.N, n, a.oact);
-          int64_t orow = m;
-          if constexpr (SUB) {
-            const int oimg = m / hw_o, orem = m - oimg * hw_o;
-            const int oi = orem / a.Wo, oj = orem - oi * a.Wo;
-            orow = ((int64_t)oimg * a.o_H + oi * a.o_sub + a.o_y) * a.o_W + oj * a.o_sub + a.o_x;
-          }
-          *reinterpret_cast<uint4*>(a.Y + orow * a.N + n) = c;
-        }
-      }
-      if (side != nullptr && p0 + PG < NP && etid) load_side(p0 + PG);
-    }
-    PF_IG_STAMP(12);
-    if constexpr (XPRE) { asm volatile("s_waitcnt lgkmcnt(0)" ::: "memory"); __builtin_amdgcn_s_barrier(); __builtin_amdgcn_sched_barrier(0); }
-    else __syncthreads();
-    PF_IG_STAMP(13);
-#ifdef PF_IG_TIMING
-    if (tm_tile == 2 && blockIdx.x == gridDim.x / 2 && tid == 0) {
-      uint32_t* out = reinterpret_cast<uint32_t*>(const_cast<bf16_t*>(a.zero));
-#pragma unroll
-      for (int k = 0; k < 14; ++k) out[k] = tmk[k];
-      out[14] = (uint32_t)__builtin_readcyclecounter();
-    }
-#endif
-  }
-
-  if (a.partial != nullptr) {
-    constexpr int nstat_max = 4;
-    const int nstat = BWD ? 2 : 4;
-    __syncthreads();
-    for (int stat = 0; stat < nstat; ++stat) {
-      const float* v = (stat == 0) ? st_s : (stat == 1 ? st_q : (stat == 2 ? st_mn : st_mx));
-#pragma unroll
-      for (int j = 0; j < 8; ++j) red[wrw * BN + wvec * 8 + j] = v[j];
-      __syncthreads();
-      for (int c = tid; c < BN; c += T) {
-        float r = red[c];
-        for (int rr = 1; rr < RPP; ++rr) {
-          const float w = red[rr * BN + c];
-          r = (stat < 2) ? (r + w) : (stat == 2 ? fminf(r, w) : fmaxf(r, w));
-        }
-        if (n0 + c < a.N) a.partial[((int64_t)g * nstat + stat) * a.N + n0 + c] = r;
-      }
-      __syncthreads();
-    }
-    (void)nstat_max;
-  }
+  static_assert(!SUB, "the SUB kernels take IgSubArgs: the overload below");
+#include "pf_igemm_kernel.inc"
+}
+
+template <int BM, int BN, int WM, int WN, int NS, int MODE, bool SUB, bool AFF, bool RMAP, bool BR>
+__global__ __launch_bounds__(64 * WM * WN) void k_igemm(const IgSubArgs a) {
+  static_assert(SUB && !AFF && !RMAP && !BR, "the class walk is compiled for the plain and the backward-data kernel");
+#include "pf_igemm_kernel.inc"
 }
 
 static IgCfg ig_pick(int M, int N, bool pro) {
@@ -590,7 +79,7 @@
 }
 
 template <int BM, int BN, int WM, int WN, int NS, int MODE, bool SUB = false, bool AFF = false, bool RMAP = false, bool BR = false>
-static int ig_launch_t(IgArgs& a, int slots, hipStream_t st) {
+static int ig_launch_t(std::conditional_t<SUB, IgSubArgs, IgArgs>& a, int slots, hipStream_t st) {
   constexpr bool BWD = (MODE == IG_BWD), PRO3 = (MODE == IG_PRO && NS == 3);
   constexpr int THREADS = 64 * WM * WN;
   a.tiles_m = (a.M + BM - 1) / BM;
@@ -598,13 +87,21 @@
   const int planned_G = a.G;
   const int grid = pf_conv_grid(slots, a.tiles_m, a.tiles_n, &a.G);
   if (planned_G > 0 && a.G != planned_G) return (int)hipErrorInvalidValue;
+  if constexpr (SUB) {
+    if (a.n_cls < 0 || a.n_cls > IG_MAX_CLS) return (int)hipErrorInvalidValue;
+    if (a.n_cls == 0) {
+      a.cls[0] = IgSubCls{a.th, a.tw, a.pad_h, a.pad_w, a.w_r0, a.w_s0, a.o_y, a.o_x, 0, 0, a.partial};
+      a.n_cls = 1;
+    }
+  }
   constexpr size_t ring = NS * (size_t)(BM + BN) * 128, ctile = (size_t)BM * (BN + 8) * 2;
   constexpr size_t base = (ring > ctile ? ring : ctile);
   const size_t lds = base + (BWD ? 4 * BN * 4 : 0) + (PRO3 ? 2 * (size_t)a.C * 4 : 0);
   if (PRO3 && a.C > CV_MAXK) return (int)hipErrorInvalidValue;
   const size_t lds_max = base + (BWD ? 4 * BN * 4 : 0) + (PRO3 ? 2 * (size_t)CV_MAXK * 4 : 0);
-  if (int e = pf_require_lds(reinterpret_cast<const void*>(&k_igemm<BM, BN, WM, WN, NS, MODE, SUB, AFF, RMAP, BR>), lds_max)) return e;
-  k_igemm<BM, BN, WM, WN, NS, MODE, SUB, AFF, RMAP, BR><<<grid, THREADS, lds, st>>>(a);
+  void (*const kern)(const std::conditional_t<SUB, IgSubArgs, IgArgs>) = &k_igemm<BM, BN, WM, WN, NS, MODE, SUB, AFF, RMAP, BR>;
+  if (int e = pf_require_lds(reinterpret_cast<const void*>(kern), lds_max)) return e;
+  kern<<<grid, THREADS, lds, st>>>(a);
   PF_LAUNCH_CHECK();
   return 0;
 }
@@ -733,44 +230,89 @@
   return stride * stride * strided_class_groups(imgs, H, Wd, C, stride);
 }
 
+static void strided_rotations(int tiles_m, int G, int n_cls, IgSubCls* cls) {
+  const int P8 = G / 8, base = tiles_m / G, rem = tiles_m % G;
+  int64_t load[512];
+  if (G > 512) { for (int c = 0; c < n_cls; ++c) cls[c].rot = 0; return; }
+  for (int p = 0; p < G; ++p) load[p] = 0;
+  for (int c = 0; c < n_cls; ++c) {
+    const int taps = cls[c].th * cls[c].tw;
+    int best = 0;
+    int64_t best_max = -1, best_sq = -1;
+    for (int r = 0; r < P8; ++r) {
+      int64_t mx = 0, sq = 0;
+      for (int p = 0; p < G; ++p) {
+        const int g = (p & 7) + 8 * (((p >> 3) + r) % P8);
+        const int64_t v = load[p] + (int64_t)taps * (base + (g < rem ? 1 : 0));
+        mx = v > mx ? v : mx;
+        sq += v * v;
+      }
+      if (best_max < 0 || mx < best_max || (mx == best_max && sq < best_sq)) { best = r; best_max = mx; best_sq = sq; }
+    }
+    cls[c].rot = best;
+    for (int p = 0; p < G; ++p) {
+      const int g = (p & 7) + 8 * (((p >> 3) + best) % P8);
+      load[p] += (int64_t)taps * (base + (g < rem ? 1 : 0));
+    }
+  }
+}
+
 static int strided_launch(const void* dY, const void* Wt, void* dX, const void* zero, int imgs, int H, int Wd, int C, int N, int R,
                           int S, int stride, int pad_h, int pad_w, int Ho, int Wo, void* stream, float* partial, const void* bn_x,
                           const float* bss, const float* bmi, int bn_act) {
   if (imgs <= 0 || H <= 0 || Wd <= 0 || Ho <= 0 || Wo <= 0 || C <= 0 || N <= 0 || (N % 64) || (C % 8) || stride < 2 || R < stride ||
-      S < stride || (H % stride) || (Wd % stride) || pad_h < 0 || pad_w < 0 || R * S > 32)
+      S < stride || (H % stride) || (Wd % stride) || pad_h < 0 || pad_w < 0 || R * S > 32 || stride * stride > IG_MAX_CLS)
     return (int)hipErrorInvalidValue;
   if (!pf_aligned16(dY) || !pf_aligned16(Wt) || !pf_aligned16(dX) || zero == nullptr) return (int)hipErrorInvalidValue;
   if ((int64_t)imgs * Ho * Wo * N >= ((int64_t)1 << 30) || (int64_t)C * R * S * N >= ((int64_t)1 << 30)) return (int)hipErrorInvalidValue;
   const int Hc = H / stride, Wc = Wd / stride;
+  IgSubArgs a;
+  static_cast<IgArgs&>(a) = ig_args_plain(1, 1);
+  a.X = (const bf16_t*)dY; a.W = (const bf16_t*)Wt; a.Y = (bf16_t*)dX; a.zero = (const bf16_t*)zero;
+  if (bn_x != nullptr) {
+    a.partial = partial; a.bx = (const bf16_t*)bn_x; a.bss = bss; a.bmi = bmi;
+    pf_act_window(bn_act, &a.b_lo, &a.b_hi);
+  }
+  a.M = imgs * Hc * Wc; a.N = C; a.C = N;
+  a.H = Ho; a.Wd = Wo; a.Ho = Hc; a.Wo = Wc; a.stride = 1;
+  a.x_bytes = (uint32_t)((int64_t)imgs * Ho * Wo * N * 2);
+  a.w_bytes = (uint32_t)((int64_t)C * R * S * N * 2);
+  a.w_rs = stride; a.w_ss = stride; a.w_S = S; a.w_taps_full = R * S;
+  a.o_sub = stride; a.o_H = H; a.o_W = Wd;
+  const int groups = strided_class_groups(imgs, H, Wd, C, stride);
+  int n = 0;
   for (int ay = 0; ay < stride; ++ay) {
     for (int ax = 0; ax < stride; ++ax) {
       const int r1 = (ay + pad_h) % stride, s1 = (ax + pad_w) % stride;
       const int th = (R - r1 + stride - 1) / stride, tw = (S - s1 + stride - 1) / stride;
       const int dmin_h = (ay + pad_h - r1) / stride - (th - 1), dmin_w = (ax + pad_w - s1) / stride - (tw - 1);
-      IgArgs a = ig_args_plain(th, tw);
-      a.X = (const bf16_t*)dY; a.W = (const bf16_t*)Wt; a.Y = (bf16_t*)dX; a.zero = (const bf16_t*)zero;
-      if (bn_x != nullptr) {
-        a.partial = partial + (int64_t)(ay * stride + ax) * strided_class_groups(imgs, H, Wd, C, stride) * 2 * C;
-        a.bx = (const bf16_t*)bn_x; a.bss = bss; a.bmi = bmi;
-        pf_act_window(bn_act, &a.b_lo, &a.b_hi);
-      }
-      a.M = imgs * Hc * Wc; a.N = C; a.C = N;
-      a.H = Ho; a.Wd = Wo; a.Ho = Hc; a.Wo = Wc; a.stride = 1; a.pad_h = -dmin_h; a.pad_w = -dmin_w;
-      a.x_bytes = (uint32_t)((int64_t)imgs * Ho * Wo * N * 2);
-      a.w_bytes = (uint32_t)((int64_t)C * R * S * N * 2);
-      a.w_r0 = (R - 1 - r1) - (th - 1) * stride; a.w_rs = stride;
-      a.w_s0 = (S - 1 - s1) - (tw - 1) * stride; a.w_ss = stride;
-      a.w_S = S; a.w_taps_full = R * S;
-      a.o_sub = stride; a.o_y = ay; a.o_x = ax; a.o_H = H; a.o_W = Wd;
-      int rc;
-      if (bn_x != nullptr)
-        rc = (C % 128 == 0) ? ig_launch_t<128, 128, 2, 2, 2, IG_BWD, true>(a, 512, (hipStream_t)stream)
-                            : ig_launch_t<128, 64, 2, 2, 2, IG_BWD, true>(a, 512, (hipStream_t)stream);
-      else
-        rc = (C % 128 == 0) ? ig_launch_t<128, 128, 2, 2, 2, IG_PLAIN, true>(a, 512, (hipStream_t)stream)
-                            : ig_launch_t<128, 64, 2, 2, 2, IG_PLAIN, true>(a, 512, (hipStream_t)stream);
-      if (rc != 0) return rc;
-    }
+      IgSubCls k;
+      k.th = th; k.tw = tw; k.pad_h = -dmin_h; k.pad_w = -dmin_w;
+      k.w_r0 = (R - 1 - r1) - (th - 1) * stride;
+      k.w_s0 = (S - 1 - s1) - (tw - 1) * stride;
+      k.o_y = ay; k.o_x = ax; k.rot = 0; k.pad_ = 0;
+      k.partial = (bn_x != nullptr) ? partial + (int64_t)(ay * stride + ax) * groups * 2 * C : nullptr;
+      int at = n++;
+      while (at > 0 && a.cls[at - 1].th * a.cls[at - 1].tw < th * tw) { a.cls[at] = a.cls[at - 1]; --at; }
+      a.cls[at] = k;
+    }
+  }
+  auto launch = [&](IgSubArgs& l) {
+    if (bn_x != nullptr)
+      return (C % 128 == 0) ? ig_launch_t<128, 128, 2, 2, 2, IG_BWD, true>(l, 512, (hipStream_t)stream)
+                            : ig_launch_t<128, 64, 2, 2, 2, IG_BWD, true>(l, 512, (hipStream_t)stream);
+    return (C % 128 == 0) ? ig_launch_t<128, 128, 2, 2, 2, IG_PLAIN, true>(l, 512, (hipStream_t)stream)
+                          : ig_launch_t<128, 64, 2, 2, 2, IG_PLAIN, true>(l, 512, (hipStream_t)stream);
+  };
+  if (pf_tuning().strided_one_launch != 0) {
+    a.n_cls = n;
+    strided_rotations((a.M + 127) / 128, groups, n, a.cls);
+    return launch(a);
+  }
+  for (int c = 0; c < n; ++c) {
+    IgSubArgs l = a;
+    l.cls[0] = a.cls[c]; l.n_cls = 1; l.G = 0;
+    if (int rc = launch(l)) return rc;
   }
   return 0;
 }
@@ -837,7 +379,10 @@
   }
   if (c.ymap) {
     a.o_sub = c.stride; a.o_y = 0; a.o_x = 0; a.o_H = c.H; a.o_W = c.Wd;
-    return wide ? ig_launch_t<128, 128, 2, 2, 2, IG_PLAIN, true>(a, 512, st) : ig_launch_t<128, 64, 2, 2, 2, IG_PLAIN, true>(a, 512, st);
+    IgSubArgs s;
+    static_cast<IgArgs&>(s) = a;
+    s.n_cls = 0;
+    return wide ? ig_launch_t<128, 128, 2, 2, 2, IG_PLAIN, true>(s, 512, st) : ig_launch_t<128, 64, 2, 2, 2, IG_PLAIN, true>(s, 512, st);
   }
   return ig_launch(a, p.ig, st);
 }
diff --git a/pocketflow_amd/csrc/pf_igemm_kernel.inc b/pocketflow_amd/csrc/pf_igemm_kernel.inc
--- /dev/null
+++ b/pocketflow_amd/csrc/pf_igemm_kernel.inc
@@ -0,0 +1,541 @@
+  constexpr bool BWD = (MODE == IG_BWD), PRO = (MODE == IG_PRO);
+  static_assert(!BR || BWD, "BR is a variant of IG_BWD");
+  static_assert(!PRO || NS == 2 || NS == 3, "the in-LDS prologue pass is written for the 2- and 3-stage rings");
+  constexpr bool PRO3 = PRO && NS == 3;
+  constexpr int NWC = WM * WN;
+  constexpr int T = 64 * NWC;
+  constexpr int TS = T;
+  constexpr int TE = T;
+  constexpr int WR = BM / WM, WC = BN / WN;
+  constexpr int JM = WR / 16, NI = WC / 16;
+  constexpr int XB = PF_IG_XB;
+  constexpr int ACH = 4 * XB, AROW = 64 * XB;
+  constexpr int AS = BM * ACH / TS, BS = BN * 8 / TS;
+  constexpr int A_BYTES = BM * AROW, B_BYTES = BN * 128, STAGE = A_BYTES + B_BYTES;
+  constexpr int CS_LD = BN + 8, CS_LD_B = BN + 8;
+  constexpr int VPR = BN / 8, RPP = TE / VPR, NP = BM / RPP;
+  static_assert(AS >= 1 && BS >= 1 && NP >= 1, "tile too small for the block");
+  constexpr int LPS = AS + BS;
+  extern __shared__ __attribute__((aligned(16))) unsigned char smem[];
+  bf16_t* Cs = reinterpret_cast<bf16_t*>(smem);
+  float* red = reinterpret_cast<float*>(smem);
+  constexpr int RING_B = NS * STAGE, CT_B = BM * CS_LD_B * 2;
+  float* bpl = reinterpret_cast<float*>(smem + (RING_B > CT_B ? RING_B : CT_B));
+  float* ssl = bpl;
+
+  const int tid = threadIdx.x, lane = tid & 63;
+  const int wave = __builtin_amdgcn_readfirstlane(tid >> 6);
+  const int swave = wave;
+  const int cwave = wave % NWC;
+  const int wm = cwave / WN, wn = cwave % WN;
+  const int l15 = lane & 15, q = lane >> 4;
+  const int srow = (swave * 64 + lane) >> 3;
+  const int schunk = (lane & 7) ^ ((lane >> 3) & 7);
+  const int srowA = (XB == 2) ? srow : ((swave * 64 + lane) >> 2);
+  const int schunkA = (XB == 2) ? schunk : ((lane & 3) ^ ((lane >> 4) & 3));
+
+  const int xcd = blockIdx.x & 7, L = blockIdx.x >> 3;
+  const int g = xcd + 8 * (L / a.tiles_n), tn = L % a.tiles_n;
+  const int n0 = tn * BN;
+  const int cch = a.C >> 6;
+  const int taps = a.th * a.tw;
+  const int nk = taps * cch;
+  const int64_t wrow = (int64_t)(SUB ? a.w_taps_full : taps) * a.C;
+#define IG_C(field) (SUB ? c_##field : a.field)
+#define IG_V(name) (SUB ? c_##name : name)
+  int c_th = 0, c_tw = 0, c_pad_h = 0, c_pad_w = 0, c_w_r0 = 0, c_w_s0 = 0, c_o_y = 0, c_o_x = 0, c_g = 0, c_nk = 0, ci = 0;
+  bool c_pointwise = false;
+  float* c_partial = nullptr;
+  int n_cls = 1;
+  if constexpr (SUB) n_cls = ig_sub_args<SUB>(a).n_cls;
+  const int hw_o = a.Ho * a.Wo;
+
+  if (BWD) {
+    for (int i = tid; i < 4 * BN; i += T) {
+      const int qq = i / BN, c = n0 + (i - qq * BN);
+      float v = 0.f;
+      if (c < a.N) v = (qq < 2) ? a.bss[qq * a.N + c] : a.bmi[(qq - 2) * a.N + c];
+      bpl[i] = v;
+    }
+  }
+
+  float st_s[8], st_q[8], st_mn[8], st_mx[8];
+#pragma unroll
+  for (int j = 0; j < 8; ++j) { st_s[j] = 0.f; st_q[j] = 0.f; st_mn[j] = INFINITY; st_mx[j] = -INFINITY; }
+  const int wvec = tid % VPR, wrw = tid / VPR;
+  const bf16_t* __restrict__ side = BWD ? a.bx : nullptr;
+  Pro pro;
+  pro_init(pro, a.act_lo, a.act_hi, a.kq, PRO ? a.slot : nullptr);
+  if (PRO3) {
+    for (int i = tid; i < 2 * a.C; i += T) ssl[i] = (i < a.C) ? pro_fold_scale(pro, a.ss[i]) : pro_fold_shift(pro, a.ss[i]);
+    __syncthreads();
+  }
+
+  const pf_rsrc_t rsX = PF_MAKE_RSRC(a.X, a.x_bytes);
+  const pf_rsrc_t rsW = PF_MAKE_RSRC(a.W, a.w_bytes);
+  constexpr uint32_t OOB = 0x80000000u;
+  uint32_t boff[BS];
+#pragma unroll
+  for (int i = 0; i < BS; ++i) {
+    const int n = n0 + i * (TS / 8) + srow;
+    boff[i] = (n < a.N) ? (uint32_t)(((int64_t)n * wrow + schunk * 8) * 2) : OOB;
+  }
+
+  const bool pointwise = a.th == 1 && a.tw == 1 && a.stride == 1 && a.pad_h == 0 && a.pad_w == 0 && a.Ho == a.H && a.Wo == a.Wd;
+  constexpr bool XPRE = !BWD && NS == 3 && 2 * STAGE >= BM * CS_LD_B * 2;
+  constexpr int RB0 = XPRE ? 2 : 0;
+  uint32_t pbase[AS], pmask[AS];
+  int s_r = 0, s_s = 0, s_cc = 0, s_ks = 0, s_tap = 0;
+  auto setup_tile = [&](int m0) {
+#pragma unroll
+    for (int i = 0; i < AS; ++i) {
+      const int m = m0 + i * (TS / ACH) + srowA;
+      pbase[i] = 0; pmask[i] = 0;
+      if (IG_V(pointwise)) {
+        if (m < a.M) { pbase[i] = (uint32_t)(m * a.C + schunkA * (16 / XB)) * (uint32_t)XB; pmask[i] = 1u; }
+      } else if (m < a.M) {
+        const int img = m / hw_o, rem = m - img * hw_o;
+        const int ho = rem / a.Wo, wo = rem - ho * a.Wo;
+        const int h0 = ho * a.stride - IG_C(pad_h), w0 = wo * a.stride - IG_C(pad_w);
+        pbase[i] = (uint32_t)(((img * a.H + h0) * a.Wd + w0) * a.C + schunkA * (16 / XB)) * (uint32_t)XB;
+        uint32_t mk = 0;
+        for (int r = 0; r < IG_C(th); ++r)
+          for (int sx = 0; sx < IG_C(tw); ++sx)
+            if ((unsigned)(h0 + r) < (unsigned)a.H && (unsigned)(w0 + sx) < (unsigned)a.Wd) mk |= 1u << (r * IG_C(tw) + sx);
+        pmask[i] = mk;
+      }
+    }
+    s_r = 0; s_s = 0; s_cc = 0; s_ks = 0; s_tap = 0;
+  };
+  auto stage = [&](int buf) {
+    unsigned char* As = smem + buf * STAGE;
+    unsigned char* Bs = As + A_BYTES;
+    const uint32_t tapoff = (uint32_t)(((s_r * a.Wd + s_s) * a.C + s_cc * 64) * XB);
+#if !PF_IG_NO_DMA
+#pragma unroll
+    for (int i = 0; i < AS; ++i) {
+      const uint32_t voff = ((pmask[i] >> s_tap) & 1u) ? (pbase[i] + tapoff) : OOB;
+      PF_BUFFER_LOAD_LDS16(rsX, As + (i * (TS / ACH) + swave * (64 / ACH)) * AROW, voff, 0);
+    }
+    uint32_t woff = (uint32_t)(s_ks * 128);
+    if constexpr (SUB) woff = (uint32_t)((((IG_C(w_r0) + s_r * a.w_rs) * a.w_S + IG_C(w_s0) + s_s * a.w_ss) * a.C + s_cc * 64) * 2);
+#pragma unroll
+    for (int i = 0; i < BS; ++i)
+      PF_BUFFER_LOAD_LDS16(rsW, Bs + (i * (TS / 8) + swave * 8) * 128, boff[i], woff);
+#else
+    (void)As; (void)Bs; (void)tapoff;
+#endif
+    ++s_ks;
+    if (++s_cc == cch) { s_cc = 0; ++s_tap; if (++s_s == IG_C(tw)) { s_s = 0; ++s_r; } }
+  };
+  bool pre = false;
+#ifdef PF_IG_TIMING
+  uint32_t tmk[16];
+  int tm_tile = -1;
+#pragma unroll
+  for (int k = 0; k < 16; ++k) tmk[k] = 0;
+#endif
+  do {
+  if constexpr (SUB) {
+    const IgSubCls& k = ig_sub_args<SUB>(a).cls[ci];
+    c_th = k.th; c_tw = k.tw; c_pad_h = k.pad_h; c_pad_w = k.pad_w;
+    c_w_r0 = k.w_r0; c_w_s0 = k.w_s0; c_o_y = k.o_y; c_o_x = k.o_x;
+    c_partial = k.partial;
+    c_g = xcd + 8 * ((L / a.tiles_n + k.rot) % (a.G >> 3));
+    c_nk = c_th * c_tw * cch;
+    c_pointwise = c_th == 1 && c_tw == 1 && a.stride == 1 && c_pad_h == 0 && c_pad_w == 0 && a.Ho == a.H && a.Wo == a.Wd;
+#pragma unroll
+    for (int j = 0; j < 8; ++j) { st_s[j] = 0.f; st_q[j] = 0.f; st_mn[j] = INFINITY; st_mx[j] = -INFINITY; }
+  }
+  for (int tm = IG_V(g); tm < a.tiles_m; tm += a.G) {
+    const int m0 = tm * BM;
+#ifdef PF_IG_TIMING
+    ++tm_tile;
+#endif
+    PF_IG_STAMP(0);
+    if (!pre) setup_tile(m0);
+
+    f32x4 acc[NI][JM];
+#pragma unroll
+    for (int i = 0; i < NI; ++i)
+#pragma unroll
+      for (int j = 0; j < JM; ++j) acc[i][j] = (f32x4){0.f, 0.f, 0.f, 0.f};
+    uint2 rr[NI][JM];
+    const bool has_r = BWD ? BR : (a.R != nullptr);
+    constexpr bool RPRE = BM * BN <= 128 * 256;
+    auto load_residual = [&]() {
+#pragma unroll
+      for (int j = 0; j < JM; ++j) {
+        const int m = m0 + wm * WR + j * 16 + l15;
+        int64_t rrow = m;
+        bool live = m < a.M;
+        if constexpr (RMAP) {
+          rrow = live ? rmap_row(m, a.rHo, a.rWo, a.rH, a.rW, a.rstride) : -1;
+          live = rrow >= 0;
+        }
+#pragma unroll
+        for (int i = 0; i < NI; ++i) {
+          const int n = n0 + wn * WC + i * 16 + q * 4;
+          rr[i][j] = make_uint2(0, 0);
+          if (live && n < a.N) rr[i][j] = *reinterpret_cast<const uint2*>(a.R + rrow * a.N + n);
+        }
+      }
+    };
+    auto add_residual = [&](auto& c) {
+#pragma unroll
+      for (int j = 0; j < JM; ++j)
+#pragma unroll
+        for (int i = 0; i < NI; ++i) {
+          c[i][j][0] += __uint_as_float(rr[i][j].x << 16); c[i][j][1] += __uint_as_float(rr[i][j].x & 0xFFFF0000u);
+          c[i][j][2] += __uint_as_float(rr[i][j].y << 16); c[i][j][3] += __uint_as_float(rr[i][j].y & 0xFFFF0000u);
+        }
+    };
+
+    int ibuf = RB0;
+    float4 ps0 = make_float4(0, 0, 0, 0), ps1 = ps0, ph0 = ps0, ph1 = ps0;
+    auto fetch_ss = [&](int cc) {
+      const float* p = a.ss + cc * 64 + schunk * 8;
+      ps0 = *reinterpret_cast<const float4*>(p); ps1 = *reinterpret_cast<const float4*>(p + 4);
+      ph0 = *reinterpret_cast<const float4*>(p + a.C); ph1 = *reinterpret_cast<const float4*>(p + a.C + 4);
+    };
+    auto transform3 = [&](int buf, int cc, int i0, int i1) {
+      const uint32_t pss = lds_addr(ssl + cc * 64 + schunk * 8);
+      float4 s0, s1, h0, h1;
+      if (i1 - i0 == 1 || i1 - i0 == 2) {
+        const uint32_t pd = lds_addr(smem + buf * STAGE + srow * 128 + (lane & 7) * 16) + (uint32_t)(i0 * (TS / 8) * 128);
+        uint4 v0, v1 = make_uint4(0, 0, 0, 0);
+        if (i1 - i0 == 1) lds_read_b128x4_1(pss, pss + (uint32_t)a.C * 4u, pd, s0, s1, h0, h1, v0);
+        else lds_read_b128x4_2(pss, pss + (uint32_t)a.C * 4u, pd, pd + (TS / 8) * 128, s0, s1, h0, h1, v0, v1);
+        pro.sc[0] = s0.x; pro.sc[1] = s0.y; pro.sc[2] = s0.z; pro.sc[3] = s0.w;
+        pro.sc[4] = s1.x; pro.sc[5] = s1.y; pro.sc[6] = s1.z; pro.sc[7] = s1.w;
+        pro.sh[0] = h0.x; pro.sh[1] = h0.y; pro.sh[2] = h0.z; pro.sh[3] = h0.w;
+        pro.sh[4] = h1.x; pro.sh[5] = h1.y; pro.sh[6] = h1.z; pro.sh[7] = h1.w;
+        lds_write_b128(pd, pro_apply(pro, v0));
+        if (i1 - i0 == 2) lds_write_b128(pd + (TS / 8) * 128, pro_apply(pro, v1));
+        return;
+      }
+      lds_read_b128x4(pss, pss + (uint32_t)a.C * 4u, s0, s1, h0, h1);
+      pro.sc[0] = s0.x; pro.sc[1] = s0.y; pro.sc[2] = s0.z; pro.sc[3] = s0.w;
+      pro.sc[4] = s1.x; pro.sc[5] = s1.y; pro.sc[6] = s1.z; pro.sc[7] = s1.w;
+      pro.sh[0] = h0.x; pro.sh[1] = h0.y; pro.sh[2] = h0.z; pro.sh[3] = h0.w;
+      pro.sh[4] = h1.x; pro.sh[5] = h1.y; pro.sh[6] = h1.z; pro.sh[7] = h1.w;
+      const uint32_t pv = lds_addr(smem + buf * STAGE + srow * 128 + (lane & 7) * 16);
+      static_assert(!PRO3 || AS == 1 || AS == 2 || AS == 4 || AS == 8, "vector count per lane");
+#pragma unroll
+      for (int i = 0; i < AS; i += 2) {
+        if (i >= i0 && i < i1) {
+          if (i + 1 < i1) {
+            uint4 v0, v1;
+            lds_read_b128x2(pv + i * (TS / 8) * 128, pv + (i + 1) * (TS / 8) * 128, v0, v1);
+            lds_write_b128(pv + i * (TS / 8) * 128, pro_apply(pro, v0));
+            lds_write_b128(pv + (i + 1) * (TS / 8) * 128, pro_apply(pro, v1));
+          } else {
+            lds_write_b128(pv + i * (TS / 8) * 128, pro_apply(pro, lds_read_b128(pv + i * (TS / 8) * 128)));
+          }
+        } else if (i + 1 >= i0 && i + 1 < i1) {
+          lds_write_b128(pv + (i + 1) * (TS / 8) * 128, pro_apply(pro, lds_read_b128(pv + (i + 1) * (TS / 8) * 128)));
+        }
+      }
+    };
+    auto transform = [&](int buf) {
+      const float rs[8] = {ps0.x, ps0.y, ps0.z, ps0.w, ps1.x, ps1.y, ps1.z, ps1.w};
+      const float rh[8] = {ph0.x, ph0.y, ph0.z, ph0.w, ph1.x, ph1.y, ph1.z, ph1.w};
+#pragma unroll
+      for (int j = 0; j < 8; ++j) { pro.sc[j] = pro_fold_scale(pro, rs[j]); pro.sh[j] = pro_fold_shift(pro, rh[j]); }
+      unsigned char* As = smem + buf * STAGE;
+#pragma unroll
+      for (int i = 0; i < AS; ++i) {
+        uint4* p = reinterpret_cast<uint4*>(As + (i * (TS / 8) + srow) * 128 + (lane & 7) * 16);
+        *p = pro_apply(pro, *p);
+      }
+    };
+    {
+#pragma unroll
+    for (int d = 0; d < NS - 1; ++d)
+      if (d < IG_V(nk)) {
+        if (d > 0 || !pre) {
+          if (PRO && !PRO3) fetch_ss(s_cc);
+          stage(ibuf);
+        }
+        ibuf = (ibuf + 1 == NS) ? 0 : ibuf + 1;
+      }
+    PF_IG_STAMP(1);
+    if (IG_V(nk) >= NS - 1) wait_vm<(NS - 2) * LPS>(); else wait_vm<0>();
+    PF_IG_STAMP(2);
+    if (PRO3) { transform3(RB0, 0, 0, AS); asm volatile("s_waitcnt lgkmcnt(0)" ::: "memory"); }
+    else if (PRO) { transform(RB0); asm volatile("s_waitcnt lgkmcnt(0)" ::: "memory"); }
+    __builtin_amdgcn_s_barrier();
+    PF_IG_STAMP(3);
+    int cbuf = RB0;
+    for (int ks = 0; ks < IG_V(nk); ++ks) {
+      const bool more = ks + NS - 1 < IG_V(nk);
+      const int tbuf = ibuf;
+      if (more) {
+        if (PRO && !PRO3) fetch_ss(s_cc);
+        stage(ibuf);
+        ibuf = (ibuf + 1 == NS) ? 0 : ibuf + 1;
+      }
+      const unsigned char* As = smem + cbuf * STAGE;
+      const unsigned char* Bs = As + A_BYTES;
+      cbuf = (cbuf + 1 == NS) ? 0 : cbuf + 1;
+      const bool tnext = PRO3 && (ks + 1 < IG_V(nk));
+      if (PRO3) {
+        if (more) wait_vm<LPS>(); else if (ks + 1 < IG_V(nk)) wait_vm<0>();
+      }
+      if (RPRE && has_r && ks == ((PRO3 && IG_V(nk) >= 2) ? IG_V(nk) - 2 : IG_V(nk) - 1)) load_residual();
+#pragma unroll
+      for (int kk = 0; kk < 2; ++kk) {
+        const int coff = (((kk * 4 + q) ^ (l15 & 7)) << 4);
+        bf16x8 wf[NI], xf[JM];
+#if PF_IG_ABLATE != 1
+#if PF_IG_FAKE_FRAGS
+#pragma unroll
+        for (int i = 0; i < NI; ++i) { uint4 u = make_uint4(lane, i, kk, 0x3f803f80u); asm volatile("" : "+v"(u.x)); wf[i] = *reinterpret_cast<const bf16x8*>(&u); }
+#pragma unroll
+        for (int j = 0; j < JM; ++j) { uint4 u = make_uint4(lane, j, kk, 0x3f803f80u); asm volatile("" : "+v"(u.x)); xf[j] = *reinterpret_cast<const bf16x8*>(&u); }
+        (void)coff;
+#else
+#pragma unroll
+        for (int i = 0; i < NI; ++i)
+          wf[i] = *reinterpret_cast<const bf16x8*>(Bs + (wn * WC + i * 16 + l15) * 128 + coff);
+#ifdef PF_IG_CODES
+        const int coffA = ((((kk * 2 + (q >> 1)) ^ ((l15 >> 2) & 3)) << 4) + (q & 1) * 8);
+#pragma unroll
+        for (int j = 0; j < JM; ++j)
+          xf[j] = ig_codes_to_bf16x8(*reinterpret_cast<const uint2*>(As + (wm * WR + j * 16 + l15) * AROW + coffA));
+#else
+#pragma unroll
+        for (int j = 0; j < JM; ++j)
+          xf[j] = *reinterpret_cast<const bf16x8*>(As + (wm * WR + j * 16 + l15) * 128 + coff);
+#endif
+#endif
+#pragma unroll
+        for (int i = 0; i < NI; ++i)
+#pragma unroll
+          for (int j = 0; j < JM; ++j)
+            acc[i][j] = __builtin_amdgcn_mfma_f32_16x16x32_bf16(wf[i], xf[j], acc[i][j], 0, 0, 0);
+        if constexpr (NI == 4 && JM == 4 && PRO3) {
+          __builtin_amdgcn_sched_group_barrier(0x100, NI + JM, 0);
+          __builtin_amdgcn_sched_group_barrier(0x008, NI * JM, 0);
+        }
+        if constexpr ((NI == 4 || NI == 2) && JM == 4 && !PRO3) {
+          if (kk == 1) {
+            __builtin_amdgcn_sched_group_barrier(0x100, NI + JM, 0);
+#pragma unroll
+            for (int i = 0; i < NI + JM; ++i) {
+              __builtin_amdgcn_sched_group_barrier(0x008, (NI * JM) / (NI + JM), 0);
+              __builtin_amdgcn_sched_group_barrier(0x100, 1, 0);
+            }
+            __builtin_amdgcn_sched_group_barrier(0x008, NI * JM - (NI + JM) * ((NI * JM) / (NI + JM)) + NI * JM, 0);
+          }
+        }
+#else
+        (void)coff; (void)wf; (void)xf;
+#endif
+        if (tnext) transform3(cbuf, ks + 1, kk * (AS / 2), (kk == 1) ? AS : (AS / 2));
+      }
+      if (!PRO3) {
+        if (more) wait_vm<(NS - 2) * LPS>(); else wait_vm<0>();
+      }
+      if (PRO && !PRO3 && more) transform(tbuf);
+      asm volatile("s_waitcnt lgkmcnt(0)" ::: "memory");
+      __builtin_amdgcn_s_barrier();
+      __builtin_amdgcn_sched_barrier(0);
+#ifdef PF_IG_TIMING
+      if (ks < 4) PF_IG_STAMP(4 + ks);
+      if (ks == IG_V(nk) - 1) PF_IG_STAMP(8);
+#endif
+    }
+    }
+
+#if PF_IG_ABLATE >= 4
+    {
+      if (a.M < 0) {
+#pragma unroll
+        for (int i = 0; i < NI; ++i)
+#pragma unroll
+          for (int j = 0; j < JM; ++j) reinterpret_cast<uint32_t*>(a.Y)[(i * JM + j) * 64 + lane] = pack_bf16x2(acc[i][j][0] + acc[i][j][1], acc[i][j][2] + acc[i][j][3]);
+      }
+      continue;
+    }
+#endif
+    {
+    if (has_r) {
+      if constexpr (RPRE) add_residual(acc);
+      else {
+#pragma unroll
+        for (int j = 0; j < JM; ++j) {
+          const int m = m0 + wm * WR + j * 16 + l15;
+          int64_t rrow = m;
+          bool live = m < a.M;
+          if constexpr (RMAP) {
+            rrow = live ? rmap_row(m, a.rHo, a.rWo, a.rH, a.rW, a.rstride) : -1;
+            live = rrow >= 0;
+          }
+#pragma unroll
+          for (int i = 0; i < NI; ++i) {
+            const int n = n0 + wn * WC + i * 16 + q * 4;
+            if (live && n < a.N) {
+              const uint2 r = *reinterpret_cast<const uint2*>(a.R + rrow * a.N + n);
+              acc[i][j][0] += __uint_as_float(r.x << 16); acc[i][j][1] += __uint_as_float(r.x & 0xFFFF0000u);
+              acc[i][j][2] += __uint_as_float(r.y << 16); acc[i][j][3] += __uint_as_float(r.y & 0xFFFF0000u);
+            }
+          }
+          __builtin_amdgcn_sched_barrier(0);
+        }
+      }
+    }
+    PF_IG_STAMP(9);
+    pre = false;
+    if constexpr (XPRE) {
+      __builtin_amdgcn_sched_barrier(0);
+      if (tm + a.G < a.tiles_m) {
+        setup_tile((tm + a.G) * BM);
+        stage(RB0);
+        pre = true;
+      }
+      __builtin_amdgcn_sched_barrier(0);
+    }
+#ifdef PF_IG_CODES
+#pragma unroll
+    for (int i = 0; i < NI; ++i)
+#pragma unroll
+      for (int j = 0; j < JM; ++j)
+#pragma unroll
+        for (int e = 0; e < 4; ++e) acc[i][j][e] *= a.kq;
+#endif
+#pragma unroll
+    for (int i = 0; i < NI; ++i)
+#pragma unroll
+      for (int j = 0; j < JM; ++j) {
+        const uint2 v = make_uint2(pack_bf16x2(acc[i][j][0], acc[i][j][1]), pack_bf16x2(acc[i][j][2], acc[i][j][3]));
+        if constexpr (XPRE) lds_write_b64(lds_addr(Cs + (wm * WR + j * 16 + l15) * CS_LD + wn * WC + i * 16 + q * 4), v);
+        else *reinterpret_cast<uint2*>(Cs + (wm * WR + j * 16 + l15) * CS_LD + wn * WC + i * 16 + q * 4) = v;
+      }
+    }
+    constexpr int PG = (NP > 8) ? 8 : NP;
+    uint4 rres[PG];
+    auto load_side = [&](int p0) {
+#pragma unroll
+      for (int p = 0; p < PG; ++p) {
+        const int m = m0 + wrw + (p0 + p) * RPP, n = n0 + wvec * 8;
+        rres[p] = make_uint4(0, 0, 0, 0);
+        if (m < a.M && n < a.N) {
+          int64_t srow = m;
+          if constexpr (SUB) {
+            const int oimg = m / hw_o, orem = m - oimg * hw_o;
+            const int oi = orem / a.Wo, oj = orem - oi * a.Wo;
+            srow = ((int64_t)oimg * a.o_H + oi * a.o_sub + IG_C(o_y)) * a.o_W + oj * a.o_sub + IG_C(o_x);
+          }
+          rres[p] = *reinterpret_cast<const uint4*>(side + srow * a.N + n);
+        }
+      }
+    };
+    constexpr bool etid = true;
+    float bpr[32];
+    if (BWD && !BR) {
+#pragma unroll
+      for (int qq = 0; qq < 4; ++qq)
+#pragma unroll
+        for (int j = 0; j < 8; ++j) bpr[qq * 8 + j] = bpl[qq * BN + wvec * 8 + j];
+    }
+    if (side != nullptr && etid) load_side(0);
+    PF_IG_STAMP(10);
+    if constexpr (XPRE) { asm volatile("s_waitcnt lgkmcnt(0)" ::: "memory"); __builtin_amdgcn_s_barrier(); __builtin_amdgcn_sched_barrier(0); }
+    else __syncthreads();
+    PF_IG_STAMP(11);
+#pragma unroll
+    for (int p0 = 0; p0 < NP; p0 += PG) {
+      u32x4_t cv[8];
+      if constexpr (XPRE && PG == 8) {
+#pragma unroll
+        for (int pp = 0; pp < PG; ++pp) lds_read_b128_nowait(lds_addr(Cs + (wrw + (p0 + pp) * RPP) * CS_LD + wvec * 8), cv[pp]);
+        lds_wait_batch8(cv);
+      } else {
+#pragma unroll
+        for (int pp = 0; pp < PG; ++pp) cv[pp] = *reinterpret_cast<const u32x4_t*>(Cs + (wrw + (p0 + pp) * RPP) * CS_LD + wvec * 8);
+      }
+#pragma unroll
+      for (int pp = 0; pp < PG; ++pp) {
+        const int p = p0 + pp;
+        const int rl = wrw + p * RPP;
+        const int m = m0 + rl, n = n0 + wvec * 8;
+        if (m < a.M && n < a.N && etid) {
+          uint4 c;
+          c = make_uint4(cv[pp][0], cv[pp][1], cv[pp][2], cv[pp][3]);
+          if (BWD) {
+            float f[8], xv[8];
+            unpack8(c, f);
+            unpack8(rres[pp], xv);
+            const float* bp = BR ? (bpl + wvec * 8) : bpr;
+            constexpr int BPS = BR ? BN : 8;
+#pragma unroll
+            for (int j = 0; j < 8; ++j) {
+              const float u = fmaf(bp[j], xv[j], bp[BPS + j]);
+              const float dy = (u > a.b_lo && u < a.b_hi) ? f[j] : 0.f;
+              st_s[j] += dy;
+              st_q[j] = fmaf(dy, (xv[j] - bp[2 * BPS + j]) * bp[3 * BPS + j], st_q[j]);
+            }
+          } else if (a.R != nullptr || a.partial != nullptr) {
+            float f[8];
+            unpack8(c, f);
+            if (a.partial != nullptr) {
+#pragma unroll
+              for (int j = 0; j < 8; ++j) {
+                st_s[j] += f[j];
+                st_q[j] = fmaf(f[j], f[j], st_q[j]);
+                st_mn[j] = pf_acc_min(st_mn[j], f[j]);
+                st_mx[j] = pf_acc_max(st_mx[j], f[j]);
+              }
+            }
+          }
+          if constexpr (AFF) c = out_affine8(c, a.oss, a.N, n, a.oact);
+          int64_t orow = m;
+          if constexpr (SUB) {
+            const int oimg = m / hw_o, orem = m - oimg * hw_o;
+            const int oi = orem / a.Wo, oj = orem - oi * a.Wo;
+            orow = ((int64_t)oimg * a.o_H + oi * a.o_sub + IG_C(o_y)) * a.o_W + oj * a.o_sub + IG_C(o_x);
+          }
+          *reinterpret_cast<uint4*>(a.Y + orow * a.N + n) = c;
+        }
+      }
+      if (side != nullptr && p0 + PG < NP && etid) load_side(p0 + PG);
+    }
+    PF_IG_STAMP(12);
+    if constexpr (XPRE) { asm volatile("s_waitcnt lgkmcnt(0)" ::: "memory"); __builtin_amdgcn_s_barrier(); __builtin_amdgcn_sched_barrier(0); }
+    else __syncthreads();
+    PF_IG_STAMP(13);
+#ifdef PF_IG_TIMING
+    if (tm_tile == 2 && blockIdx.x == gridDim.x / 2 && tid == 0) {
+      uint32_t* out = reinterpret_cast<uint32_t*>(const_cast<bf16_t*>(a.zero));
+#pragma unroll
+      for (int k = 0; k < 14; ++k) out[k] = tmk[k];
+      out[14] = (uint32_t)__builtin_readcyclecounter();
+    }
+#endif
+  }
+
+  if (a.partial != nullptr) {
+    constexpr int nstat_max = 4;
+    const int nstat = BWD ? 2 : 4;
+    __syncthreads();
+    for (int stat = 0; stat < nstat; ++stat) {
+      const float* v = (stat == 0) ? st_s : (stat == 1 ? st_q : (stat == 2 ? st_mn : st_mx));
+#pragma unroll
+      for (int j = 0; j < 8; ++j) red[wrw * BN + wvec * 8 + j] = v[j];
+      __syncthreads();
+      for (int c = tid; c < BN; c += T) {
+        float r = red[c];
+        for (int rr = 1; rr < RPP; ++rr) {
+          const float w = red[rr * BN + c];
+          r = (stat < 2) ? (r + w) : (stat == 2 ? fminf(r, w) : fmaxf(r, w));
+        }
+        if (n0 + c < a.N) IG_C(partial)[((int64_t)IG_V(g) * nstat + stat) * a.N + n0 + c] = r;
+      }
+      __syncthreads();
+    }
+    (void)nstat_max;
+  }
+  } while (SUB && ++ci < n_cls);
+#undef IG_C
+#undef IG_V
```

Result: no change. 11650, median of 6 (+0.3%).
